# zubair-irshad/articulated-object-nerf

Measured on AMD Instinct MI355X. Metric: rays/sec (64c+128f samples), higher is better.
Workload: dtype f32; 1 GPU; sapien-single-scene vanilla NeRF full-frame render 640x480, 65 coarse + 193 fine evals/ray, 307200 rays per GPU per step, randomized=False, white_bkgd=True; rays_per_gpu=307200, evals_per_ray=258, exchange=none

## Files before the change

articulated-object-nerf_amd/_lib.py:

```python
from __future__ import annotations

import ctypes as C
import os

import torch

_PKG = os.path.dirname(os.path.abspath(__file__))
LIB_PATH = os.environ.get("AON_HIP_LIB") or os.path.join(_PKG, "libaon_hip.so")

if not os.path.exists(LIB_PATH):
    raise ImportError(
        f"{LIB_PATH} not found: the HIP kernels are the product path and there is no CPU/eager fallback. "
        "Build them with `python articulated-object-nerf_amd/build.py` (needs /opt/rocm/bin/hipcc)."
    )

lib = C.CDLL(LIB_PATH)

_p, _i, _l, _f = C.c_void_p, C.c_int, C.c_int64, C.c_float
_PATH = ([_p, _p, _p, _l]
         + [_f, _f, _i, _i]
         + [_p, _p, _l]
         + [_p] * 6
         + [_p, _l, _p])
_VANILLA, _ART, _GENERAL = [_p] * 2, [_p] * 4, [_p] * 3
# ... 18 lines not shown
    head, tail = _BWD
    vanilla = _VANILLA * 2 + head + _PER_LEVEL + tail
    art = _ART + head + _PER_LEVEL + _LATENTS + _PER_LEVEL + _LATENTS + tail
    frozen = _ART + head + _PER_LEVEL + _LATENTS + tail + _OPTS
    sigs = {"aon_render_bwd": vanilla, "aon_render_bwd_ex": vanilla + _OPTS, "aon_art_render_bwd": art, "aon_art_render_bwd_ex": art + _OPTS,
            "aon_art_render_bwd_latents": frozen, "aon_art_render_bwd_inputs": frozen + _RAY_GRADS,
            "aon_grender_bwd": _GENERAL + head + _PER_LEVEL + tail + _OPTS}
    return {name: (_i, args) for name, args in sigs.items()}


_SIGS = {
    **_path_sigs(),
    **_bwd_sigs(),
    "aon_abi_version": (_i, []),
    "aon_last_error": (C.c_char_p, []),
    "aon_raygen": (_i, [_p, _i, _i, _f, _l, _l, _p, _p, _p, _p]),
    "aon_train_loss_fwd": (_i, [_p, _p, _p, _l, _p, _p, _f, _p, _p, _p]),
    "aon_train_loss_bwd": (_i, [_p, _p, _p, _l, _p, _p, _f, _p, _p, _p, _p, _p]),
    "aon_ray_directions": (_i, [_i, _i, _f, _p, _p]),
    "aon_get_rays": (_i, [_p, _p, _l, _p, _p, _p, _p]),
    "aon_ray_radii": (_i, [_p, _p, _i, _i, _p, _p]),
    "aon_cast_rays": (_i, [_p, _p, _p, _l, _i, _p, _p]),
    "aon_sample_along_rays": (_i, [_p, _p, _l, _i, _f, _f, _p, _p, _p, _p]),
    "aon_pos_enc": (_i, [_p, _l, _i, _i, _p, _p]),
    "aon_mlp_packed_bytes": (_l, []),
    "aon_pack_vanilla_mlp": (_i, [_p, _p, _p]),
    "aon_mlp_fwd": (_i, [_p, _p, _p, _p, _p, _l, _i, _p, _p]),
    "aon_mlp_fwd_enc": (_i, [_p, _p, _p, _l, _i, _p, _p]),
    "aon_composite": (_i, [_p, _i, _p, _i, _p, _p, _l, _i, _i, _i, _p, _p, _p, _p, _p]),
    "aon_sample_pdf": (_i, [_p, _p, _l, _p, _p, _l, _l, _p, _p, _p]),
    "aon_art_packed_bytes": (_l, []),
    "aon_art_small_bytes": (_l, []),
    "aon_pack_art_mlp": (_i, [_p, _p, _p]),
    "aon_art_prepare": (_i, [_p, _p, _p, _p, _p, _p]),
    "aon_pack_art_mlp_deg": (_i, [_p, _i, _i, _i, _p, _p]),
    "aon_art_prepare_deg": (_i, [_p, _p, _p, _p, _i, _i, _i, _p, _p]),
    "aon_pack_art_mlp_bwd_deg": (_i, [_p, _i, _i, _i, _p, _p]),
    "aon_art_mlp_fwd": (_i, [_p, _p, _p, _p, _p, _p, _l, _i, _p, _p]),
    "aon_art_mlp_fwd_pos": (_i, [_p, _p, _p, _p, _l, _i, _p, _p]),
    "aon_train_plane_rows": (_l, []),
    "aon_bwd_packed_bytes": (_l, []),
    "aon_wgrad_workspace_bytes": (_l, []),
    "aon_pack_vanilla_mlp_bwd": (_i, [_p, _p, _p]),
    "aon_train_mask_bytes": (_l, [_l]),
    "aon_mlp_fwd_train": (_i, [_p, _p, _p, _p, _p, _l, _i, _p, _p, _p, _p]),
    "aon_composite_bwd": (_i, [_p, _p, _p, _p, _p, _p, _l, _i, _i, _i, _p, _p]),
    "aon_mlp_bwd_chain": (_i, [_p, _p, _p, _p, _p, _l, _p]),
    "aon_vanilla_wgrad": (_i, [_p, _p, _p, _l, _p, _p, _l, _p, _p]),
    "aon_wgrad_plan": (_i, [_i, _l, _i, _p, _i, _p]),
    "aon_wgrad_plan_segment": (_i, [_i, _l, _i, _i, _i, _p]),
    "aon_wgrad_kind_bench": (_i, [_i, _i, _p, _p, _i, _l, _p, _l, _p]),
    "aon_art_train_plane_rows": (_l, []),
    "aon_art_train_mask_bytes": (_l, [_l]),
    "aon_art_bwd_packed_bytes": (_l, []),
    "aon_pack_art_mlp_bwd": (_i, [_p, _p, _p]),
    "aon_art_mlp_fwd_train": (_i, [_p, _p, _p, _p, _p, _p, _l, _i, _p, _p, _p, _p]),
    "aon_art_bwd_chain": (_i, [_p, _p, _p, _p, _p, _p, _p, _l, _p]),
    "aon_art_wgrad": (_i, [_p, _p, _p, _p, _l, _p, _p, _p, _p, _p, _p, _p, _p, _p, _l, _p, _p]),
    "aon_art_wgrad_deg": (_i, [_p, _p, _p, _p, _l, _p, _p, _p, _p, _p, _p, _p, _p, _p, _l, _p, _i, _i, _i, _p]),
    "aon_set_bottleneck_fold": (_i, [_i]),
    "aon_get_bottleneck_fold": (_i, []),
    "aon_stream_is_folded": (_i, [_p]),
    "aon_stream_form": (_i, [_p]),
    "aon_declare_stream_form": (_i, [_p, _i]),
    "aon_adam_step": (_i, [_p, _p, _p, _p, _l, C.c_double, C.c_double, C.c_double, C.c_double, _l, _p]),
    "aon_code_library_fwd": (_i, [_p, _p, _p, _p, _p, _p]),
    "aon_code_library_bwd": (_i, [_p, _p, _p, _p, _p, _p]),
    "aon_ssim_workspace_bytes": (_l, [_i, _p, _p]),
    "aon_ssim": (_i, [_i, _p, _p, _p, _p, _p, _l, _p, _p]),
    "aon_density_grid": (_i, [_p, _p, _p, _p, _l, _l, _i, _p, _p]),
    "aon_art_density_grid": (_i, [_p, _p, _p, _p, _p, _l, _l, _i, _p, _p]),
    "aon_marching_cubes_workspace_bytes": (_l, [_p]),
    "aon_marching_cubes_count": (_i, [_p, _p, _f, _p, _l, _p, _p]),
    "aon_marching_cubes": (_i, [_p, _p, _f, _p, _p, _p, _l, _p, _l, _p, _l, _p]),
    "aon_occupancy_bytes": (_l, [_p]),
    "aon_occupancy_build": (_i, [_p, _p, _f, _i, _p, _p]),
    "aon_render_occ_workspace_bytes": (_l, [_l, _p]),
    "aon_render_stop_workspace_bytes": (_l, [_l, _p]),
    "aon_art_pack_step": (_i, [_p, _p, _p, _p, _p, _i, _i, _i, _p, _p, _p, _p, _p, _p, _p]),
    "aon_vanilla_pack_step": (_i, [_p, _p, _i, _i, _i, _p, _p, _p, _p, _p]),
    "aon_set_bwd_early_heads": (_i, [_i]),
    "aon_set_view_bias": (_i, [_i]),
    "aon_get_view_bias": (_i, []),
    "aon_view_bias": (_i, [_p, _p, _l, _p, _p]),
    "aon_set_bwd_overlap": (_i, [_i]),
    "aon_set_fwd_overlap": (_i, [_i]),
    "aon_set_fwd_merge": (_i, [_i]),
    "aon_set_bwd_merge": (_i, [_i]),
    "aon_set_wgrad_probe": (_i, [_p]),
    "aon_train_workspace_bytes": (_l, [_l, _i, _i]),
    "aon_train_scratch_bytes": (_l, [_l, _i, _i]),
    "aon_profile_begin": (_i, []),
    "aon_profile_end": (_i, [C.POINTER(C.c_double), C.POINTER(C.c_int64), C.POINTER(C.c_int64)]),
    "aon_profile_class": (_i, [_i, C.POINTER(C.c_double), C.POINTER(C.c_int64), C.POINTER(C.c_int64)]),
    "aon_composite_pdf": (_i, [_p, _p, _p, _l, _i, _i, _p, _l, _p, _p, _p, _p, _p, _p]),
    "aon_set_coarse_fusion": (_i, [_i]),
    "aon_render_workspace_bytes": (_l, [_l]),
    "aon_render_opts_init": (None, [_p]),
    "aon_pack_vanilla_mlp_deg": (_i, [_p, _i, _i, _i, _p, _p]),
    "aon_pack_vanilla_mlp_bwd_deg": (_i, [_p, _i, _i, _i, _p, _p]),
    "aon_sample_along_rays_ex": (_i, [_p, _p, _l, _i, _f, _f, _i, _f, _f, _p, _p, _p, _p]),
    "aon_composite_ex": (_i, [_p, _i, _p, _i, _p, _p, _l, _i, _i, _i, _p, _p, _p, _p, _p, _p]),
    "aon_sample_pdf_n": (_i, [_p, _p, _l, _p, _p, _l, _l, _i, _i, _i, _p, _p, _p]),
    "aon_render_workspace_bytes_ex": (_l, [_l, _p]),
    "aon_train_workspace_bytes_ex": (_l, [_l, _i, _i, _p]),
    "aon_train_scratch_bytes_ex": (_l, [_l, _i, _i, _p]),
    "aon_train_scratch_bytes_latents": (_l, [_l, _i, _p]),
    "aon_train_scratch_bytes_inputs": (_l, [_l, _i, _p]),
    "aon_mlp_geometry_init": (None, [_p]),
    "aon_gmlp_param_count": (_i, [_p]),
    "aon_gmlp_workspace_bytes": (_l, [_p, _l]),
    "aon_gmlp_fwd": (_i, [_p, _p, _p, _p, _l, _i, _p, _p, _p, _l, _p]),
    "aon_grender_workspace_bytes": (_l, [_p, _l, _p]),
    "aon_grender_train_workspace_bytes": (_l, [_p, _l, _i, _p]),
    "aon_grender_train_scratch_bytes": (_l, [_p, _l, _i, _p]),
    "aon_ray_limits_box": (_i, [_p, _p, _l, _p, _p, _p, _p, _p]),
    "aon_ray_limits_workspace_bytes": (_l, [_l]),
    "aon_ray_limits": (_i, [_p, _p, _l, _p, _p, _p, _p, _p, _p, _l, _p]),
    "aon_sample_along_rays_bounds": (_i, [_p, _p, _l, _i, _p, _p, _i, _p, _p, _p, _p]),
}


class MlpGeometryC(C.Structure):
    _fields_ = [(n, C.c_int32) for n in ("min_deg_point", "max_deg_point", "deg_view", "netdepth", "netwidth", "netdepth_condition",
                                         "netwidth_condition", "skip_layer", "input_ch", "input_ch_view", "num_rgb_channels",
                                         "num_density_channels")]


class RenderOptsC(C.Structure):
    _fields_ = [("num_coarse_samples", C.c_int32), ("num_fine_samples", C.c_int32), ("lindisp", C.c_int32),
                ("inv_near", C.c_float), ("inv_far", C.c_float), ("noise_std", C.c_float),
                ("noise_c", C.c_void_p), ("noise_f", C.c_void_p),
                ("rgb_scale", C.c_float), ("rgb_shift", C.c_float), ("sigma_bias", C.c_float),
                ("min_deg_point", C.c_int32), ("max_deg_point", C.c_int32), ("deg_view", C.c_int32)]


class OccupancyC(C.Structure):
    _fields_ = [("bits", C.c_void_p), ("cells", C.c_int64 * 3), ("lo", C.c_float * 3), ("step", C.c_float * 3)]


class RayGradsC(C.Structure):
    _fields_ = [("rays_o", C.c_void_p), ("viewdirs", C.c_void_p), ("g_rays_o", C.c_void_p), ("g_rays_d", C.c_void_p), ("g_viewdirs", C.c_void_p)]


class RayBoundsC(C.Structure):
    _fields_ = [("near_ray", C.c_void_p), ("far_ray", C.c_void_p), ("live", C.c_void_p)]


class SceneObjectC(C.Structure):
    _fields_ = [("rot", C.c_float * 9), ("centre", C.c_float * 3), ("lo", C.c_float * 3), ("hi", C.c_float * 3)]


def _ext_sigs():
    head, tail = _BWD
    return {"aon_render_bwd_inputs": (_i, _VANILLA * 2 + head + _PER_LEVEL + tail + _OPTS + _RAY_GRADS),
            "aon_train_scratch_bytes_inputs_vanilla": (_l, [_l, _i] + _OPTS)}


_EXT_SIGS = _ext_sigs()

_SCENE_SIGS = {
    "aon_scene_pairs_workspace_bytes": (_l, [_l, _i]),
    "aon_scene_pairs": (_i, [_p, _p, _p, _l] + [_p, _i] + [_p, _l] + [_p] * 8 + [_p]),
    "aon_scene_composite": (_i, [_p] * 4 + [_l, _i, _l, _i, _i, _i] + [_p] + [_p] * 5 + [_p]),
}

# ... 54 lines not shown
```

articulated-object-nerf_amd/csrc/aon_capi.hip:

```cpp
#include "aon_capi_util.h"

namespace aon {
namespace capi __attribute__((visibility("hidden"))) {

thread_local char g_err[256] = "";

int fail(int code, const char* msg) {
  std::snprintf(g_err, sizeof(g_err), "%s", msg);
  return code;
}

int check(hipError_t e, const char* where) {
  if (e == hipSuccess) return AON_OK;
  std::snprintf(g_err, sizeof(g_err), "%s: %s", where, hipGetErrorString(e));
  return AON_E_HIP_BASE - (int)e;
}

const char* const kFormsMsg = "two of the packed buffers of this call were made in different forms (aon_set_bottleneck_fold changed between the pack / prepare calls), "
                              "or one of them was never packed or declared by this process (a copy: aon_declare_stream_form)";
const char* const kNullBwdMsg = "packed_bwd is NULL (= literal planes) while the process default is the folded form: pass the transposed stream the chain ran with";

Profiler g_prof;

std::atomic<int> g_fuse_coarse{1};
std::atomic<int> g_view_bias{1};

const char* make_geo(const aon_render_opts* o, Geo& g, bool general_engine) {
  aon_render_opts d;
  aon_render_opts_init(&d);
  if (o) d = *o;
  if (d.num_coarse_samples < 2 || d.num_coarse_samples > 1023) return "num_coarse_samples must be in [2, 1023]";
  if (d.num_fine_samples < 1) return "num_fine_samples must be >= 1";
  g.Sc = d.num_coarse_samples + 1; g.nf = d.num_fine_samples; g.Sf = g.Sc + g.nf;
  g.default_sizes = g.Sc == kSc && g.Sf == kSf;
  if (!g.default_sizes && aon::sample_pdf_n_lds_bytes(g.Sc - 1, g.nf, g.Sc, nullptr) > 64 * 1024) return "num_coarse_samples / num_fine_samples too large for the per-ray LDS image";
  g.lindisp = d.lindisp != 0; g.inv_near = d.inv_near; g.inv_far = d.inv_far;
  g.noise[0] = d.noise_c; g.noise[1] = d.noise_f; g.noise_std = d.noise_std;
  g.rgb_scale = d.rgb_scale; g.rgb_shift = d.rgb_shift; g.sigma_bias = d.sigma_bias;
  g.min_deg = d.min_deg_point; g.max_deg = d.max_deg_point; g.deg_view = d.deg_view;
  if (general_engine) { g.min_deg = 0; g.max_deg = 10; g.deg_view = 4; g.other_degrees = false; return nullptr; }
  if (g.max_deg < g.min_deg || g.max_deg - g.min_deg > 10 || g.deg_view < 0 || g.deg_view > 4)
    return "the fused kernels hold up to 10 position and 4 view frequency levels (other degrees: aon_grender_*)";
  g.other_degrees = !(g.min_deg == 0 && g.max_deg == 10 && g.deg_view == 4);
  return nullptr;
}

}
}

using namespace aon::capi;

extern "C" {

int aon_abi_version(void) { return AON_ABI_VERSION; }

const char* aon_last_error(void) { return g_err; }

int aon_raygen(const float* c2w_host, int H, int W, float focal, int64_t pix_begin, int64_t pix_end, float* rays_o,
               float* viewdirs, float* rays_d, void* stream) {
  if (!c2w_host || !rays_o || !viewdirs) return fail(AON_E_INVALID, "aon_raygen: null pointer");
  if (H <= 0 || W <= 0 || !(focal > 0.f) || pix_begin < 0 || pix_end < pix_begin || pix_end > (int64_t)H * W)
    return fail(AON_E_INVALID, "aon_raygen: bad geometry");
  return check(aon::launch_raygen(c2w_host, H, W, focal, nullptr, pix_begin, pix_end, rays_o, viewdirs, rays_d,
                                  (hipStream_t)stream), "aon_raygen");
}

int aon_train_loss_fwd(const float* rgb_coarse, const float* rgb_fine, const float* target, int64_t n, const float* const* latents_host, const int* latent_len_host,
                       float reg_scale, float* stats, float* loss, void* stream) {
  if (!rgb_fine || !target || !stats || !loss) return fail(AON_E_INVALID, "aon_train_loss_fwd: null pointer");
  if (n <= 0) return fail(AON_E_INVALID, "aon_train_loss_fwd: bad size");
  for (int k = 0; k < 3 && latents_host; ++k)
    if (latents_host[k] && (!latent_len_host || latent_len_host[k] <= 0)) return fail(AON_E_INVALID, "aon_train_loss_fwd: bad latent length");
  return check(aon::launch_train_loss(false, rgb_coarse, rgb_fine, target, n, latents_host, latent_len_host, reg_scale, stats, loss, nullptr, nullptr, nullptr, nullptr,
                                      (hipStream_t)stream), "aon_train_loss_fwd");
}

int aon_train_loss_bwd(const float* rgb_coarse, const float* rgb_fine, const float* target, int64_t n, const float* const* latents_host, const int* latent_len_host,
                       float reg_scale, const float* grad_loss, float* d_rgb_coarse, float* d_rgb_fine, float* const* d_latents_host, void* stream) {
  if (!rgb_fine || !target || !grad_loss || !d_rgb_fine) return fail(AON_E_INVALID, "aon_train_loss_bwd: null pointer");
  if (n <= 0) return fail(AON_E_INVALID, "aon_train_loss_bwd: bad size");
  if ((rgb_coarse == nullptr) != (d_rgb_coarse == nullptr)) return fail(AON_E_INVALID, "aon_train_loss_bwd: coarse level input / gradient mismatch");
  for (int k = 0; k < 3 && latents_host; ++k)
    if (latents_host[k] && (!latent_len_host || latent_len_host[k] <= 0)) return fail(AON_E_INVALID, "aon_train_loss_bwd: bad latent length");
  return check(aon::launch_train_loss(true, rgb_coarse, rgb_fine, target, n, latents_host, latent_len_host, reg_scale, nullptr, nullptr, grad_loss, d_rgb_coarse, d_rgb_fine,
                                      d_latents_host, (hipStream_t)stream), "aon_train_loss_bwd");
}

int aon_view_bias(const void* packed, const float* viewdirs, int64_t n_rays, float* view_bias, void* stream) {
  if (n_rays < 0) return fail(AON_E_INVALID, "aon_view_bias: bad size");
  if (n_rays == 0) return AON_OK;
  if (!packed || !viewdirs || !view_bias) return fail(AON_E_INVALID, "aon_view_bias: null pointer");
  if (aon::stream_form(packed) != aon::kFormFolded) return fail(AON_E_INVALID, "aon_view_bias: the stream was packed in the literal form (aon_set_bottleneck_fold)");
  return check(aon::launch_view_bias(static_cast<const char*>(packed), viewdirs, n_rays, view_bias, (hipStream_t)stream), "aon_view_bias");
}

int aon_ray_directions(int H, int W, float focal, float* directions, void* stream) {
  if (H <= 0 || W <= 0 || !(focal > 0.f) || !directions) return fail(AON_E_INVALID, "aon_ray_directions: bad argument");
  return check(aon::launch_ray_directions(H, W, focal, directions, (hipStream_t)stream), "aon_ray_directions");
}

int aon_get_rays(const float* directions, const float* c2w_host, int64_t n, float* rays_o, float* viewdirs, float* rays_d,
                 void* stream) {
  if (n < 0) return fail(AON_E_INVALID, "aon_get_rays: bad size");
  if (n == 0) return AON_OK;
  if (!directions || !c2w_host || !rays_o || !viewdirs) return fail(AON_E_INVALID, "aon_get_rays: null pointer");
  return check(aon::launch_raygen(c2w_host, 1, (int)(n > INT32_MAX ? INT32_MAX : n), 1.0f, directions, 0, n, rays_o, viewdirs,
                                  rays_d, (hipStream_t)stream), "aon_get_rays");
}
// ... 489 lines not shown
int64_t aon_marching_cubes_workspace_bytes(const int64_t* dims3_host) {
  if (const char* msg = mc_dims_bad(dims3_host)) return fail(AON_E_INVALID, (std::string("aon_marching_cubes_workspace_bytes: ") + msg).c_str());
  return aon::mc_workspace_bytes(dims3_host);
}
int aon_marching_cubes_count(const float* grid, const int64_t* dims3_host, float level, void* workspace, int64_t workspace_bytes, int64_t* counts2_host,
                             void* stream) {
  if (const char* msg = mc_dims_bad(dims3_host)) return fail(AON_E_INVALID, (std::string("aon_marching_cubes_count: ") + msg).c_str());
  if (!grid || !workspace || !counts2_host) return fail(AON_E_INVALID, "aon_marching_cubes_count: null pointer");
  if (reinterpret_cast<uintptr_t>(workspace) & 15) return fail(AON_E_INVALID, "aon_marching_cubes_count: workspace is not 16-byte aligned");
  if (workspace_bytes < aon::mc_workspace_bytes(dims3_host)) return fail(AON_E_WORKSPACE, "aon_marching_cubes_count: workspace too small");
  if (int rc = check(aon::launch_mc_count(grid, dims3_host, level, workspace, (hipStream_t)stream, counts2_host), "aon_marching_cubes_count"); rc != AON_OK)
    return rc;
  if (counts2_host[0] > INT32_MAX)
    return fail(AON_E_INVALID, "aon_marching_cubes_count: more than 2^31 - 1 vertices (faces hold int32 vertex ids): use a coarser grid");
  return AON_OK;
}
int aon_marching_cubes(const float* grid, const int64_t* dims3_host, float level, const float* lo3_host, const float* step3_host, void* workspace,
                       int64_t workspace_bytes, float* verts, int64_t n_verts, int32_t* faces, int64_t n_faces, void* stream) {
  if (const char* msg = mc_dims_bad(dims3_host)) return fail(AON_E_INVALID, (std::string("aon_marching_cubes: ") + msg).c_str());
  if (!grid || !workspace || !lo3_host || !step3_host) return fail(AON_E_INVALID, "aon_marching_cubes: null pointer");
  if (n_verts < 0 || n_faces < 0 || n_verts > INT32_MAX) return fail(AON_E_INVALID, "aon_marching_cubes: bad output size");
  if ((n_verts > 0 && !verts) || (n_faces > 0 && !faces)) return fail(AON_E_INVALID, "aon_marching_cubes: null output");
  if (reinterpret_cast<uintptr_t>(workspace) & 15) return fail(AON_E_INVALID, "aon_marching_cubes: workspace is not 16-byte aligned");
  if (workspace_bytes < aon::mc_workspace_bytes(dims3_host)) return fail(AON_E_WORKSPACE, "aon_marching_cubes: workspace too small");
  return check(aon::launch_mc(grid, dims3_host, level, lo3_host, step3_host, workspace, verts, n_verts, faces, n_faces, (hipStream_t)stream),
               "aon_marching_cubes");
}

int aon_profile_begin(void) {
  std::lock_guard<std::mutex> lk(g_prof.mu);
  g_prof.on = true; g_prof.used = 0; g_prof.recs.clear();
  for (int c = 0; c < kNumClasses; ++c) g_prof.units[c] = 0;
  return AON_OK;
}

int aon_profile_end(double* mlp_ms, int64_t* mlp_launches, int64_t* mlp_samples) {
  std::lock_guard<std::mutex> lk(g_prof.mu);
  g_prof.on = false;
  for (int c = 0; c < kNumClasses; ++c) { g_prof.last_ms[c] = 0.0; g_prof.last_launches[c] = 0; g_prof.last_units[c] = g_prof.units[c]; }
  for (const auto& r : g_prof.recs) {
    hipError_t e = hipEventSynchronize(r.stop);
    if (e != hipSuccess) return check(e, "aon_profile_end");
    float ms = 0.f;
    e = hipEventElapsedTime(&ms, r.start, r.stop);
    if (e != hipSuccess) return check(e, "aon_profile_end");
    g_prof.last_ms[r.cls] += ms;
    g_prof.last_launches[r.cls] += 1;
  }
  if (mlp_ms) *mlp_ms = g_prof.last_ms[kMlpFwd];
  if (mlp_launches) *mlp_launches = g_prof.last_launches[kMlpFwd];
  if (mlp_samples) *mlp_samples = g_prof.last_units[kMlpFwd];
  g_prof.used = 0; g_prof.recs.clear();
  return AON_OK;
}

int aon_profile_class(int cls, double* ms, int64_t* launches, int64_t* units) {
  if (cls < 0 || cls >= kNumClasses) return fail(AON_E_INVALID, "aon_profile_class: unknown kernel class");
  std::lock_guard<std::mutex> lk(g_prof.mu);
  if (ms) *ms = g_prof.last_ms[cls];
  if (launches) *launches = g_prof.last_launches[cls];
  if (units) *units = g_prof.last_units[cls];
  return AON_OK;
}

int aon_set_bottleneck_fold(int on) {
  aon::set_fold_default(on);
  return AON_OK;
}
int aon_get_bottleneck_fold(void) { return aon::fold_default(); }
int aon_stream_is_folded(const void* packed) { return aon::stream_form(packed) == aon::kFormFolded ? 1 : 0; }
int aon_stream_form(const void* packed) { return aon::stream_form(packed); }
int aon_declare_stream_form(const void* packed, int form) {
  if (!packed || (form != aon::kFormLiteral && form != aon::kFormFolded)) return fail(AON_E_INVALID, "aon_declare_stream_form: null pointer or form not 0 / 1");
  aon::set_stream_form(packed, form);
  return AON_OK;
}

int aon_set_view_bias(int on) {
  g_view_bias.store(on ? 1 : 0, std::memory_order_relaxed);
  return AON_OK;
}

int aon_get_view_bias(void) { return g_view_bias.load(std::memory_order_relaxed); }

int64_t aon_art_packed_bytes(void) { return aon::art_stream_bytes(); }
int64_t aon_art_small_bytes(void) { return aon::art_small_bytes(); }

int aon_pack_art_mlp(const float* const* params_host, void* packed, void* stream) {
  return aon_pack_art_mlp_deg(params_host, 0, 10, 4, packed, stream);
}
int aon_pack_art_mlp_deg(const float* const* params_host, int min_deg_point, int max_deg_point, int deg_view, void* packed, void* stream) {
  if (const char* bad = art_degrees_ok(min_deg_point, max_deg_point, deg_view)) return fail(AON_E_INVALID, bad);
  if (!params_host || !packed) return fail(AON_E_INVALID, "aon_pack_art_mlp: null pointer");
  for (int i = 0; i < 40; ++i)
    if (!params_host[i]) return fail(AON_E_INVALID, "aon_pack_art_mlp: null parameter pointer");
  if (reinterpret_cast<uintptr_t>(packed) & 15) return fail(AON_E_INVALID, "aon_pack_art_mlp: packed must be 16-byte aligned");
  return check(aon::launch_pack_art(params_host, static_cast<float*>(packed), (hipStream_t)stream, max_deg_point - min_deg_point, deg_view),
               "aon_pack_art_mlp");
}

int aon_art_prepare(const float* const* params_host, const float* shape, const float* appearance, const float* articulation,
                    void* small, void* stream) {
  return aon_art_prepare_deg(params_host, shape, appearance, articulation, 0, 10, 4, small, stream);
}
int aon_art_prepare_deg(const float* const* params_host, const float* shape, const float* appearance, const float* articulation,
                        int min_deg_point, int max_deg_point, int deg_view, void* small, void* stream) {
  if (const char* bad = art_degrees_ok(min_deg_point, max_deg_point, deg_view)) return fail(AON_E_INVALID, bad);
  if (!params_host || !shape || !appearance || !articulation || !small) return fail(AON_E_INVALID, "aon_art_prepare: null pointer");
  for (int i = 0; i < 40; ++i)
    if (!params_host[i]) return fail(AON_E_INVALID, "aon_art_prepare: null parameter pointer");
  if (reinterpret_cast<uintptr_t>(small) & 15) return fail(AON_E_INVALID, "aon_art_prepare: small must be 16-byte aligned");
  return check(aon::launch_prepare_art(params_host, shape, appearance, articulation, static_cast<float*>(small), (hipStream_t)stream, min_deg_point,
                                       max_deg_point - min_deg_point, deg_view), "aon_art_prepare");
}

int aon_art_pack_step(const float* const* params_coarse_host, const float* const* params_fine_host, const float* shape, const float* appearance,
                      const float* articulation, int min_deg_point, int max_deg_point, int deg_view, void* packed_coarse, void* small_coarse,
                      void* packed_bwd_coarse, void* packed_fine, void* small_fine, void* packed_bwd_fine, void* stream_) {
  if (const char* bad = art_degrees_ok(min_deg_point, max_deg_point, deg_view)) return fail(AON_E_INVALID, bad);
  if (!params_coarse_host || !params_fine_host || !shape || !appearance || !articulation || !packed_coarse || !small_coarse || !packed_fine || !small_fine)
    return fail(AON_E_INVALID, "aon_art_pack_step: null pointer");
  for (int i = 0; i < 40; ++i)
    if (!params_coarse_host[i] || !params_fine_host[i]) return fail(AON_E_INVALID, "aon_art_pack_step: null parameter pointer");
  for (const void* p : {(const void*)packed_coarse, (const void*)small_coarse, (const void*)packed_fine, (const void*)small_fine, (const void*)packed_bwd_coarse, (const void*)packed_bwd_fine})
    if (reinterpret_cast<uintptr_t>(p) & 15) return fail(AON_E_INVALID, "aon_art_pack_step: buffers must be 16-byte aligned");
  hipStream_t stream = (hipStream_t)stream_;
  const int Lp = max_deg_point - min_deg_point, Lv = deg_view;
  const float* const* P[2] = {params_coarse_host, params_fine_host};
  float* fwd[2] = {static_cast<float*>(packed_coarse), static_cast<float*>(packed_fine)};
  float* sm[2] = {static_cast<float*>(small_coarse), static_cast<float*>(small_fine)};
  float* bwd[2] = {static_cast<float*>(packed_bwd_coarse), static_cast<float*>(packed_bwd_fine)};
  const int form = aon::fold_default();
  const bool folded = form == aon::kFormFolded;
  if (folded) {
    aon::FoldGemm jobs[4];
    int n = 0;
    for (int l = 0; l < 2; ++l) jobs[n++] = aon::art_fold_job_fwd(P[l], fwd[l], Lv);
    for (int l = 0; l < 2; ++l)
      if (bwd[l]) jobs[n++] = aon::art_fold_job_bwd(P[l], bwd[l], Lv);
    if (int rc = check(aon::launch_fold_gemms(jobs, n, stream), "aon_art_pack_step")) return rc;
  }
  if (int rc = check(aon::launch_pack_prepare_art2(P, shape, appearance, articulation, fwd, sm, stream, min_deg_point, Lp, Lv, form), "aon_art_pack_step")) return rc;
  if (bwd[0] && bwd[1]) return check(aon::launch_pack_art_bwd2(P, bwd, stream, Lp, Lv, form), "aon_art_pack_step");
  for (int l = 0; l < 2; ++l)
    if (bwd[l])
      if (int rc = check(aon::launch_pack_art_bwd(P[l], bwd[l], stream, Lp, Lv, folded), "aon_art_pack_step")) return rc;
  return AON_OK;
}

int aon_art_mlp_fwd(const void* packed, const void* small, const float* rays_o, const float* rays_d, const float* viewdirs,
                    const float* t_vals, int64_t n_rays, int S, float* raw, void* stream) {
  if (n_rays < 0 || S < 1) return fail(AON_E_INVALID, "aon_art_mlp_fwd: bad size");
  if (n_rays == 0) return AON_OK;
  if (!packed || !small || !rays_o || !rays_d || !viewdirs || !t_vals || !raw) return fail(AON_E_INVALID, "aon_art_mlp_fwd: null pointer");
  if (forms_differ(packed, small)) return fail(AON_E_INVALID, kFormsMsg);
  MlpTimer timer((hipStream_t)stream, n_rays * S);
  return check(aon::launch_art_mlp_fwd(static_cast<const char*>(packed), static_cast<const float*>(small), rays_o, rays_d, viewdirs,
                                       t_vals, n_rays, S, raw, (hipStream_t)stream), "aon_art_mlp_fwd");
}

int aon_art_mlp_fwd_pos(const void* packed, const void* small, const float* pos, const float* viewdirs_enc, int64_t n_rays, int S,
                        float* raw, void* stream) {
  if (n_rays < 0 || S < 1) return fail(AON_E_INVALID, "aon_art_mlp_fwd_pos: bad size");
  if (n_rays == 0) return AON_OK;
  if (!packed || !small || !pos || !viewdirs_enc || !raw) return fail(AON_E_INVALID, "aon_art_mlp_fwd_pos: null pointer");
  if (forms_differ(packed, small)) return fail(AON_E_INVALID, kFormsMsg);
// ... 6 lines not shown
```

articulated-object-nerf_amd/csrc/aon_capi_render.hip:

```cpp
#include "aon_capi_util.h"

using namespace aon::capi;

namespace {

struct Ws {
  float* t_c;
  float* w_c;
  float* t_f;
  float* raw;
  float* coords; float* enc; float* venc;
  float* vbias;
  char* occ;
  char* stop;
  int64_t bytes;
};

Ws carve(char* base, int64_t n, const Geo& g, bool occ = false, bool stop = false) {
  Ws w{};
  int64_t off = 0;
  w.t_c = reinterpret_cast<float*>(base + off); off += align_up(n * g.Sc * 4, 256);
  w.w_c = reinterpret_cast<float*>(base + off); off += align_up(n * g.Sc * 4, 256);
  w.t_f = reinterpret_cast<float*>(base + off); off += align_up(n * g.Sf * 4, 256);
  w.raw = reinterpret_cast<float*>(base + off); off += align_up(n * g.Sf * 16, 256);
  if (g.other_degrees) {
    w.coords = reinterpret_cast<float*>(base + off); off += align_up(n * g.Sf * 12, 256);
    w.enc = reinterpret_cast<float*>(base + off); off += align_up(n * g.Sf * (int64_t)aon::kPosEnc * 4, 256);
    w.venc = reinterpret_cast<float*>(base + off); off += align_up(n * (int64_t)aon::kViewEnc * 4, 256);
  } else {
    w.vbias = reinterpret_cast<float*>(base + off); off += align_up(n * (int64_t)aon::kCondWidth * 4, 256);
  }
  if (occ) { w.occ = base + off; off += aon::occ_list_bytes(n * g.Sf); }
  if (stop) { w.stop = base + off; off += aon::occ_stop_state_bytes(n); }
  w.bytes = off;
  return w;
}

}

extern "C" {

static int64_t workspace_query(int64_t n_rays, const aon_render_opts* opts, bool occ, bool stop) {
  Geo g;
  if (const char* bad = make_geo(opts, g)) return fail(AON_E_INVALID, bad);
  if (n_rays < 1) n_rays = 1;
  if (occ && n_rays > INT32_MAX / g.Sf) n_rays = INT32_MAX / g.Sf;
  return carve(nullptr, n_rays, g, occ, stop).bytes;
}
int64_t aon_render_workspace_bytes_ex(int64_t n_rays, const aon_render_opts* opts) { return workspace_query(n_rays, opts, false, false); }
int64_t aon_render_workspace_bytes(int64_t n_rays) { return aon_render_workspace_bytes_ex(n_rays, nullptr); }


struct NetRef {
  bool articulated;
  const void* packed;
  const float* small;
};
struct Nets { NetRef c, f; };
static Nets vanilla_nets(const void* packed_coarse, const void* packed_fine) {
  return {{false, packed_coarse, nullptr}, {false, packed_fine, nullptr}};
}
static Nets art_nets(const void* packed_coarse, const void* small_coarse, const void* packed_fine, const void* small_fine) {
  return {{true, packed_coarse, static_cast<const float*>(small_coarse)}, {true, packed_fine, static_cast<const float*>(small_fine)}};
}

struct OccCtx {
  aon::OccGrid grid;
  int64_t* tally;
  bool rounds;
  float tau_stop;
  int R;
  int32_t* stop_dev;
};

static hipError_t launch_net(const NetRef& net, const float* o, const float* d, const float* v, const float* t, int64_t n, int S,
                             float* raw, hipStream_t stream, const Geo* g = nullptr, const Ws* w = nullptr, const OccCtx* occ = nullptr,
                             int level = 0, const uint8_t* live = nullptr) {
  if (g && g->other_degrees) {
    if (hipError_t e = aon::launch_cast_rays(t, o, d, n, S, w->coords, stream); e != hipSuccess) return e;
    if (hipError_t e = aon::launch_pos_enc(w->coords, n * S, g->min_deg, g->max_deg, w->enc, stream, aon::kPosEnc, 10); e != hipSuccess) return e;
    if (hipError_t e = aon::launch_pos_enc(v, n, 0, g->deg_view, w->venc, stream, aon::kViewEnc, 4); e != hipSuccess) return e;
    MlpTimer timer(stream, n * S);
    return aon::launch_mlp_fwd_enc(static_cast<const char*>(net.packed), w->enc, w->venc, n, S, raw, stream);
  }
  const float* vbias = nullptr;
  if (w && w->vbias && g_view_bias.load(std::memory_order_relaxed) != 0 && aon::stream_form(net.packed) == aon::kFormFolded) {
    const hipError_t e = net.articulated ? aon::launch_art_view_bias(static_cast<const char*>(net.packed), net.small, v, n, w->vbias, stream)
                                         : aon::launch_view_bias(static_cast<const char*>(net.packed), v, n, w->vbias, stream);
    if (e != hipSuccess) return e;
    vbias = w->vbias;
  }
  const int* idx = nullptr;
  const int64_t* count = nullptr;
  auto compact = [&](int s0, int s1, const int* stop) {
    const int64_t starts[2] = {0, n};
    const aon::OccCompact c{&occ->grid, starts, 1, S, s0, s1, o, d, t, live, stop};
    return aon::launch_occ_compact(c, raw, w->occ, (n * S + 1023) / 1024, occ->tally ? occ->tally + level : nullptr, &idx, &count, stream);
  };
  if (occ && occ->rounds) {
    if (hipError_t e = aon::launch_occ_stop_init(w->stop, n, S, stream); e != hipSuccess) return e;
    const int R = occ->R < S ? occ->R : S;
    const aon::ActParams ap = g->act(net.articulated, level, 0);
    for (int s0 = 0; s0 < S; s0 += R) {
      const int s1 = s0 + R < S ? s0 + R : S;
      if (hipError_t e = compact(s0, s1, aon::occ_stop_state(w->stop, n).stop); e != hipSuccess) return e;
      {
        MlpTimer timer(stream, n * (s1 - s0));
        const hipError_t e = net.articulated ? aon::launch_art_mlp_fwd_gather(static_cast<const char*>(net.packed), net.small, o, d, v, t, n, S, raw, stream,
                                                                              vbias, idx, count, n * (s1 - s0))
                                             : aon::launch_mlp_fwd_gather(static_cast<const char*>(net.packed), o, d, v, t, n, S, raw, stream, vbias, idx,
                                                                          count, n * (s1 - s0));
        if (e != hipSuccess) return e;
      }
      if (s1 < S)
        if (hipError_t e = aon::launch_occ_depth(raw, t, d, n, S, s0, s1, ap, occ->tau_stop, w->stop, stream); e != hipSuccess) return e;
    }
    return hipSuccess;
  }
  if (occ) {
    if (hipError_t e = compact(0, S, nullptr); e != hipSuccess) return e;
    MlpTimer timer(stream, n * S);
    if (net.articulated)
      return aon::launch_art_mlp_fwd_gather(static_cast<const char*>(net.packed), net.small, o, d, v, t, n, S, raw, stream, vbias, idx, count);
    return aon::launch_mlp_fwd_gather(static_cast<const char*>(net.packed), o, d, v, t, n, S, raw, stream, vbias, idx, count);
  }
  MlpTimer timer(stream, n * S);
  if (net.articulated)
    return aon::launch_art_mlp_fwd(static_cast<const char*>(net.packed), net.small, o, d, v, t, n, S, raw, stream, vbias);
  return aon::launch_mlp_fwd(static_cast<const char*>(net.packed), o, d, v, t, n, S, raw, stream, vbias);
}

static int render_impl(const char* who, const NetRef& coarse, const NetRef& fine, const PathCall& c, const OccCtx* occ = nullptr) {
  Geo g;
  if (const char* bad = make_geo(c.opts, g)) return fail(AON_E_INVALID, bad);
  if (int rc = path_call_check(who, c, g, true)) return rc == kPathEmpty ? AON_OK : rc;
  const int64_t n_rays = c.n_rays;
  const int num_levels = c.num_levels;
  const hipStream_t stream = c.stream;
  auto bad = [&](const char* what) { return fail(AON_E_INVALID, (std::string(who) + ": " + what).c_str()); };
  if (!coarse.packed || (num_levels == 2 && !fine.packed)) return bad("null pointer");
  if (coarse.articulated && (!coarse.small || (num_levels == 2 && !fine.small))) return bad("null latent block");
  if (coarse.articulated && (forms_differ(coarse.packed, coarse.small) || (num_levels == 2 && forms_differ(fine.packed, fine.small)))) return fail(AON_E_INVALID, kFormsMsg);
  const bool art = coarse.articulated;
  if (art) g.other_degrees = false;
  const bool fuse_coarse = num_levels == 2 && g.default_sizes && g_fuse_coarse.load(std::memory_order_relaxed) != 0;
  const bool with_occ = occ != nullptr;
  const bool with_stop = with_occ && occ->rounds;

  int64_t chunk = n_rays;
  if (with_occ && chunk > INT32_MAX / g.Sf) chunk = INT32_MAX / g.Sf;
  if (carve(nullptr, chunk, g, with_occ, with_stop).bytes > c.workspace_bytes) {
    const int64_t per_ray = (int64_t)(g.Sc + g.Sc + g.Sf + 4 * g.Sf + (g.other_degrees ? (3 + aon::kPosEnc) * g.Sf + aon::kViewEnc : aon::kCondWidth) +
                                      (with_occ ? g.Sf + 2 * (g.Sf / 1024 + 1) : 0) + (with_stop ? 2 : 0)) * 4;
    const int64_t slack = (g.other_degrees ? 7 * 256 : 5 * 256) + (with_occ ? 4 * 256 : 0) + (with_stop ? 2 * 256 : 0);
    chunk = (c.workspace_bytes - slack) / per_ray;
    while (chunk > 0 && carve(nullptr, chunk, g, with_occ, with_stop).bytes > c.workspace_bytes) --chunk;
    if (chunk < 1) return fail(AON_E_WORKSPACE, with_stop ? "render: workspace smaller than aon_render_stop_workspace_bytes(1)"
                                                : with_occ ? "render: workspace smaller than aon_render_occ_workspace_bytes(1)"
                                                         : "render: workspace smaller than aon_render_workspace_bytes(1)");
  }
  const Ws w = carve(static_cast<char*>(c.workspace), chunk, g, with_occ, with_stop);
  if (with_occ && occ->tally) {
    if (int rc = check(hipMemsetAsync(occ->tally, 0, 2 * sizeof(int64_t), stream), who); rc != AON_OK) return rc;
  }

  for (int64_t r0 = 0; r0 < n_rays; r0 += chunk) {
    const int64_t n = n_rays - r0 < chunk ? n_rays - r0 : chunk;
    const float* o = c.rays_o + r0 * 3;
    const float* d = c.rays_d + r0 * 3;
    const float* v = c.viewdirs + r0 * 3;
    const float* uu = c.u_stride ? c.u + r0 * c.u_stride : c.u;
    const float* near_ray = c.bounds ? c.bounds->near_ray + r0 : nullptr;
    const float* far_ray = c.bounds ? c.bounds->far_ray + r0 : nullptr;
    const uint8_t* live = c.bounds && c.bounds->live ? c.bounds->live + r0 : nullptr;
    int rc;
    {
      KTimer timer(kSampleT, stream, n);
      rc = check(aon::launch_sample_along_rays(o, d, n, g.Sc, c.near_, c.far_, c.t_rand ? c.t_rand + r0 * g.Sc : nullptr, w.t_c, nullptr, stream,
                                               g.lindisp, g.inv_near, g.inv_far, near_ray, far_ray), who);
    }
    if (rc) return rc;
    rc = check(launch_net(coarse, o, d, v, w.t_c, n, g.Sc, w.raw, stream, &g, &w, occ, 0, live), who);
    if (rc) return rc;
    if (with_stop && occ->stop_dev) {
      rc = check(aon::launch_occ_stop_store(w.stop, 0, occ->stop_dev + r0 * 2, n, 2, stream), who);
      if (rc) return rc;
    }
    if (fuse_coarse) {
      KTimer timer(kCompositePdf, stream, n);
      rc = check(aon::launch_composite_pdf(w.raw, w.t_c, d, n, c.white_bkgd, g.act(art, 0, r0), uu, c.u_stride, c.rgb[0] + r0 * 3,
                                           c.acc[0] + r0, c.depth[0] + r0, nullptr, w.t_f, stream), who);
    } else {
      KTimer timer(kComposite, stream, n);
      rc = check(aon::launch_composite(w.raw, 4, w.raw + 3, 4, w.t_c, d, n, g.Sc, c.white_bkgd, g.act(art, 0, r0), c.rgb[0] + r0 * 3, c.acc[0] + r0,
                                       c.depth[0] + r0, num_levels == 2 ? w.w_c : nullptr, stream), who);
    }
    if (rc) return rc;
    if (num_levels == 1) continue;
    if (!fuse_coarse) {
      KTimer timer(kSamplePdf, stream, n);
      rc = check(g.default_sizes ? aon::launch_sample_pdf(nullptr, w.w_c + 1, kSc, w.t_c, uu, c.u_stride, n, nullptr, w.t_f, stream)
                                 : aon::launch_sample_pdf_n(nullptr, w.w_c + 1, g.Sc, w.t_c, uu, c.u_stride, n, g.Sc - 1, g.nf, g.Sc, nullptr,
                                                            w.t_f, stream), who);
      if (rc) return rc;
    }
    rc = check(launch_net(fine, o, d, v, w.t_f, n, g.Sf, w.raw, stream, &g, &w, occ, 1, live), who);
    if (rc) return rc;
    if (with_stop && occ->stop_dev) {
      rc = check(aon::launch_occ_stop_store(w.stop, 0, occ->stop_dev + r0 * 2 + 1, n, 2, stream), who);
      if (rc) return rc;
    }
    {
      KTimer timer(kComposite, stream, n);
      rc = check(aon::launch_composite(w.raw, 4, w.raw + 3, 4, w.t_f, d, n, g.Sf, c.white_bkgd, g.act(art, 1, r0), c.rgb[1] + r0 * 3, c.acc[1] + r0,
                                       c.depth[1] + r0, nullptr, stream), who);
    }
    if (rc) return rc;
  }
  return AON_OK;
}

int64_t aon_occupancy_bytes(const int64_t* cells3_host) {
  if (const char* msg = occ_cells_bad(cells3_host)) return fail(AON_E_INVALID, (std::string("aon_occupancy_bytes: ") + msg).c_str());
  return (cells3_host[0] * cells3_host[1] * cells3_host[2] + 31) / 32 * 4;
}
int aon_occupancy_build(const float* density, const int64_t* dims3_host, float threshold, int dilate, uint32_t* bits, void* stream) {
  if (!dims3_host) return fail(AON_E_INVALID, "aon_occupancy_build: null dims");
  const int64_t cells[3] = {dims3_host[0] - 1, dims3_host[1] - 1, dims3_host[2] - 1};
  if (const char* msg = occ_cells_bad(cells)) return fail(AON_E_INVALID, (std::string("aon_occupancy_build: every dimension must be >= 2; ") + msg).c_str());
  if (dilate < 0 || dilate > 8) return fail(AON_E_INVALID, "aon_occupancy_build: dilate must be in [0, 8]");
  if (threshold != threshold) return fail(AON_E_INVALID, "aon_occupancy_build: threshold is NaN");
  if (!density || !bits) return fail(AON_E_INVALID, "aon_occupancy_build: null pointer");
  return check(aon::launch_occ_build(density, dims3_host, threshold, dilate, bits, (hipStream_t)stream), "aon_occupancy_build");
}
static const char* occ_opts_bad(const aon_render_opts* opts, bool art, const float* t_rand) {
  Geo g;
  if (const char* bad = make_geo(opts, g)) return bad;
  if (t_rand) return "occupancy rendering is inference only: t_rand (randomized sampling) is refused";
  if (g.noise_std > 0.f && (g.noise[0] || g.noise[1])) return "occupancy rendering is inference only: density noise is refused";
  if (!art && g.other_degrees) return "occupancy rendering needs the default encoding degrees (0, 10, 4) of the vanilla network";
  return nullptr;
}
int64_t aon_render_occ_workspace_bytes(int64_t n_rays, const aon_render_opts* opts) { return workspace_query(n_rays, opts, true, false); }

// ... 140 lines not shown
```

articulated-object-nerf_amd/csrc/aon_capi_util.h:

```cpp
#pragma once
#include "../../include/aon_hip.h"
#include "aon_launch.h"

#include <atomic>
#include <cmath>
#include <cstdio>
#include <cstdlib>
#include <cstring>
#include <mutex>
#include <string>
#include <vector>

namespace aon {
namespace capi __attribute__((visibility("hidden"))) {

extern thread_local char g_err[256];

int fail(int code, const char* msg);
int check(hipError_t e, const char* where);

constexpr int kSc = 65, kSf = 193;

extern const char* const kFormsMsg;
extern const char* const kNullBwdMsg;
inline bool forms_differ(const void* a, const void* b) {
  return a && b && (aon::stream_form(a) != aon::stream_form(b) || aon::stream_form(a) == aon::kFormUnknown);
}

extern std::atomic<int> g_fuse_coarse;
extern std::atomic<int> g_view_bias;

enum KClass { kMlpFwd = AON_PROF_MLP_FWD, kBwdChain = AON_PROF_BWD_CHAIN, kWgrad = AON_PROF_WGRAD, kComposite = AON_PROF_COMPOSITE,
              kSamplePdf = AON_PROF_SAMPLE_PDF, kCompositeBwd = AON_PROF_COMPOSITE_BWD, kCompositePdf = AON_PROF_COMPOSITE_PDF, kSampleT = AON_PROF_SAMPLE_T,
              kNumClasses = AON_PROF_NUM_CLASSES };

struct Profiler {
  std::mutex mu;
  bool on = false;
  struct Rec { int cls; hipEvent_t start, stop; };
  std::vector<hipEvent_t> pool;
  size_t used = 0;
  std::vector<Rec> recs;
  int64_t units[kNumClasses] = {};
  double last_ms[kNumClasses] = {};
  int64_t last_launches[kNumClasses] = {};
  int64_t last_units[kNumClasses] = {};
};
extern Profiler g_prof;

struct KTimer {
  hipEvent_t stop = nullptr;
  hipStream_t stream;
  KTimer(int cls, hipStream_t s, int64_t units) : stream(s) {
    std::lock_guard<std::mutex> lk(g_prof.mu);
    if (!g_prof.on) return;
    while (g_prof.used + 2 > g_prof.pool.size()) {
      hipEvent_t e;
      if (hipEventCreate(&e) != hipSuccess) return;
      g_prof.pool.push_back(e);
    }
    hipEvent_t start = g_prof.pool[g_prof.used];
    stop = g_prof.pool[g_prof.used + 1];
    g_prof.used += 2;
    g_prof.recs.push_back({cls, start, stop});
    g_prof.units[cls] += units;
    (void)hipEventRecord(start, stream);
  }
  ~KTimer() { if (stop) (void)hipEventRecord(stop, stream); }
};
struct MlpTimer : KTimer {
  MlpTimer(hipStream_t s, int64_t samples) : KTimer(kMlpFwd, s, samples) {}
};

inline int64_t align_up(int64_t x, int64_t a) { return (x + a - 1) / a * a; }

struct Geo {
  int Sc, Sf, nf;
  bool default_sizes;
  int lindisp; float inv_near, inv_far;
  const float* noise[2]; float noise_std;
  float rgb_scale, rgb_shift, sigma_bias;
  int min_deg, max_deg, deg_view;
  bool other_degrees;
  int S(int l) const { return l == 0 ? Sc : Sf; }
  aon::ActParams act(bool art, int level, int64_t ray0) const {
    aon::ActParams ap{art ? AON_ACT_ARTICULATED : AON_ACT_VANILLA, rgb_scale, rgb_shift, sigma_bias, nullptr, noise_std};
    if (noise[level] && noise_std > 0.f) ap.noise = noise[level] + ray0 * S(level);
    return ap;
  }
};

const char* make_geo(const aon_render_opts* o, Geo& g, bool general_engine = false);

inline const char* occ_cells_bad(const int64_t* cells3) {
  if (!cells3) return "null cell counts";
  for (int a = 0; a < 3; ++a)
    if (cells3[a] < 1 || cells3[a] > (int64_t)1 << 24) return "every cell count must be in [1, 2^24]";
  if (cells3[0] > ((int64_t)1 << 40) / cells3[1] / cells3[2]) return "grid too large (more than 2^40 cells)";
  return nullptr;
}
inline const char* occ_grid_bad(const aon_occupancy* occ, aon::OccGrid& G) {
  if (!occ || !occ->bits) return "null occupancy grid";
  if (const char* msg = occ_cells_bad(occ->cells)) return msg;
  G.bits = occ->bits;
  for (int a = 0; a < 3; ++a) {
    if (!std::isfinite(occ->lo[a]) || !std::isfinite(occ->step[a]) || !(occ->step[a] > 0.f)) return "occupancy lo must be finite and step finite and > 0";
    G.cells[a] = occ->cells[a]; G.lo[a] = occ->lo[a]; G.step[a] = occ->step[a];
    const float span = (float)occ->cells[a] * occ->step[a];
    G.hi[a] = occ->lo[a] + span;
    if (!std::isfinite(G.hi[a])) return "occupancy box not finite";
  }
  return nullptr;
}
// ... 58 lines not shown
```

articulated-object-nerf_amd/csrc/aon_launch.h:

```cpp
#pragma once
#include "aon_common.h"
#include "aon_fold.h"

namespace aon {

int num_cus();
hipError_t launch_pack_vanilla(const float* const* params, float* packed, hipStream_t stream, int pos_levels = 10, int view_levels = 4, bool fold_done = false);
void vanilla_fold_jobs_fwd(const float* const* params, float* packed, int view_levels, FoldGemm jobs[2]);
hipError_t launch_mlp_fwd(const char* packed, const float* rays_o, const float* rays_d, const float* viewdirs,
                          const float* t_vals, int64_t n_rays, int S, float* raw, hipStream_t stream, const float* view_bias = nullptr);
hipError_t launch_view_bias(const char* packed, const float* viewdirs, int64_t n_rays, float* out, hipStream_t stream);
hipError_t launch_view_bias_raw(const float* chunk, const float* bias_vec, const float* viewdirs, int64_t n_rays, float* out, hipStream_t stream);
hipError_t launch_mlp_fwd_enc(const char* packed, const float* samples_enc, const float* viewdirs_enc, int64_t n_rays,
                              int S, float* raw, hipStream_t stream);
hipError_t launch_mlp_fwd_gather(const char* packed, const float* rays_o, const float* rays_d, const float* viewdirs, const float* t_vals,
                                 int64_t n_rays, int S, float* raw, hipStream_t stream, const float* view_bias, const int* idx, const int64_t* count,
                                 int64_t max_listed = 0);
hipError_t launch_mlp_fwd_train(const char* packed, const float* rays_o, const float* rays_d, const float* viewdirs,
                                const float* t_vals, int64_t n_rays, int S, float* raw, float* planes, void* masks,
                                hipStream_t stream, int64_t np_total = 0, const float* view_bias = nullptr);
hipError_t launch_mlp_fwd_train2(const TrainSeg* segs, int nsegs, hipStream_t stream);
hipError_t launch_mlp_fwd_train_enc(const char* packed, const float* samples_enc, const float* viewdirs_enc, int64_t n_rays, int S, float* raw,
                                    float* planes, void* masks, hipStream_t stream, int64_t np_total = 0);
hipError_t launch_density_grid(const char* packed, const int64_t* dims, const float* lo, const float* step, int64_t g_begin, int64_t g_end,
                               int act, float* out, hipStream_t stream);

int64_t art_stream_bytes();
int64_t art_small_bytes();
hipError_t launch_pack_art(const float* const* params, float* packed, hipStream_t stream, int pos_levels = 10, int view_levels = 4, bool fold_done = false);
FoldGemm art_fold_job_fwd(const float* const* params, float* packed, int view_levels);
hipError_t launch_prepare_art(const float* const* params, const float* shape, const float* app, const float* art,
                              float* small, hipStream_t stream, int min_deg = 0, int pos_levels = 10, int view_levels = 4);
hipError_t launch_pack_prepare_art2(const float* const* const params[2], const float* shape, const float* app, const float* art, float* const packed[2],
                                    float* const small[2], hipStream_t stream, int min_deg, int pos_levels, int view_levels, int form);
hipError_t launch_art_mlp_fwd(const char* packed, const float* small, const float* rays_o, const float* rays_d,
                              const float* viewdirs, const float* t_vals, int64_t n_rays, int S, float* raw,
                              hipStream_t stream, const float* view_bias = nullptr);
hipError_t launch_art_view_bias(const char* packed, const float* small, const float* viewdirs, int64_t n_rays, float* out, hipStream_t stream);
hipError_t launch_art_mlp_fwd_pos(const char* packed, const float* small, const float* pos, const float* viewdirs_enc,
                                  int64_t n_rays, int S, float* raw, hipStream_t stream);
hipError_t launch_art_mlp_fwd_gather(const char* packed, const float* small, const float* rays_o, const float* rays_d, const float* viewdirs,
                                     const float* t_vals, int64_t n_rays, int S, float* raw, hipStream_t stream, const float* view_bias,
                                     const int* idx, const int64_t* count, int64_t max_listed = 0);
hipError_t launch_art_mlp_fwd_train(const char* packed, const float* small, const float* rays_o, const float* rays_d,
                                    const float* viewdirs, const float* t_vals, int64_t n_rays, int S, float* raw, float* planes,
                                    void* masks, hipStream_t stream, int64_t np_total = 0, const float* view_bias = nullptr);
hipError_t launch_art_mlp_fwd_train2(const TrainSeg* segs, int nsegs, hipStream_t stream);
hipError_t launch_art_density_grid(const char* packed, const float* small, const int64_t* dims, const float* lo, const float* step,
                                   int64_t g_begin, int64_t g_end, int act, float* out, hipStream_t stream);

struct WgLayerDesc;
struct HeadDesc;
struct HeadOut;
struct ReduceArgs;

struct WgAux {
  hipStream_t stream;
  hipEvent_t fork, join;
};

enum : int { kWgAll = 0, kWgEarly = 1, kWgRest = 2 };

struct VanillaWgDeferred;
struct ArtWgDeferred;
constexpr int kVanillaWgDeferredBytes = 4096;
constexpr int kArtWgDeferredBytes = 4096;

hipError_t launch_composite_bwd(const float* raw, const float* t_vals, const float* dirs, const float* g_rgb, const float* g_acc,
                                const float* g_depth, int64_t n_rays, int S, int white_bkgd, const ActParams& ap, float* d_raw,
                                hipStream_t stream);
void vanilla_fold_jobs_bwd(const float* const* params, float* packed, int view_size, FoldGemm jobs[2]);
hipError_t launch_pack_vanilla_bwd(const float* const* params, float* packed, hipStream_t stream, int pos_size = 63, int view_size = 27, bool fold_done = false);
int64_t bwd_stream_bytes();
hipError_t launch_mlp_bwd_chain(const char* packed_bwd, const char* packed_fwd, const float* d_raw, const void* masks,
                                float* dplanes, int64_t Np, hipStream_t stream);
hipError_t launch_mlp_bwd_chain2(const ChainSeg* segs, int nsegs, hipStream_t stream);
int64_t wgrad_workspace_bytes();
float* wgrad_fold_tmp(float* ws);
void set_wgrad_probe(long long* buf);
hipError_t run_wgrad_plan(const WgLayerDesc* layers, int nlayers, const HeadDesc* heads, int nheads, const HeadOut* outs, const int* out_head, int nouts,
                          const float* planes, const float* dplanes, int rows_total, int64_t Np, float* ws, hipStream_t stream, const WgAux* aux,
                          int phase, int n_early, hipEvent_t wait_first, ReduceArgs* defer_reduce, int* defer_blocks);
hipError_t launch_wgrad_reduce2(const ReduceArgs& a0, int n0, const ReduceArgs& a1, int n1, hipStream_t stream);
hipError_t launch_wgrad_kind_bench(int kind, int nlayers, const float* planes, const float* dplanes, int rows_total, int64_t Np, float* ws,
                                   float* out_scratch, hipStream_t stream);
hipError_t launch_vanilla_wgrad(const float* planes, const float* dplanes, const float* d_raw, int64_t Np, float* const* grads,
                                float* ws, hipStream_t stream, const WgAux* aux, const void* packed_bwd, int phase = kWgAll, hipEvent_t wait_first = nullptr,
                                VanillaWgDeferred* defer = nullptr);
hipError_t launch_vanilla_wgrad_post2(const VanillaWgDeferred* d0, const VanillaWgDeferred* d1, hipStream_t stream);
int vanilla_wgrad_deferred_bytes();
int wgrad_plan_describe(bool art, int64_t Np, int cus, int32_t* out6, int max_jobs, int64_t* ws_bytes);
int wgrad_plan_segment(bool art, int64_t Np, int cus, int j, int wg, int32_t* begin_end);

// ... 115 lines not shown
```

articulated-object-nerf_amd/csrc/aon_mlp.hip:

```cpp
#include "aon_pass.h"

namespace aon {

struct VanillaNet {
  static constexpr int kSlotBytes = kPairSlotBytes;
  static constexpr bool kPair = true;
  static constexpr int kNumChunks = aon::kNumChunks;
  static constexpr int chunk_bytes(int c) { return aon::chunk_bytes(c); }
};
struct VanillaFoldNet {
  static constexpr int kSlotBytes = kPairSlotBytes;
  static constexpr bool kPair = true;
  static constexpr int kNumChunks = aon::kNumChunksF;
  static constexpr int chunk_bytes(int c) { return aon::chunk_bytes_f(c); }
};
struct VanillaFoldVbNet {
  static constexpr int kSlotBytes = kPairSlotBytes;
  static constexpr bool kPair = true;
  static constexpr int kNumChunks = aon::kNumChunksF - 1;
  static constexpr int chunk_bytes(int c) { return aon::chunk_bytes_f(c < kChFView ? c : c + 1); }
  static constexpr int skip_before(int c) { return c == kChFView ? kSmallChunkBytes : 0; }
};

struct PackArgs {
  const float* p[kNumVanillaParams];
};

template <bool FOLD>
__global__ void pack_vanilla_kernel(PackArgs a, float* __restrict__ packed, int L, int Lv) {
  const int P = 3 + 6 * L, V = 3 + 6 * Lv;
  const int64_t idx = (int64_t)blockIdx.x * blockDim.x + threadIdx.x;
  constexpr int64_t stream_floats = kStreamBytes / 4;
  constexpr int64_t used_floats = FOLD ? kStreamBytesF / 4 : stream_floats;
  const float* Wf = packed + kFoldTmpOff / 4;
  if (idx >= stream_floats + kSmallFloats) return;
  if (idx >= used_floats && idx < stream_floats) {
    if (idx >= used_floats + 128 * 256 + 128) packed[idx] = 0.f;
    return;
  }
  if (idx >= stream_floats) {
    const int s = (int)(idx - stream_floats);
    float v = 0.f;
    if (s < kSmBiasBott) v = a.p[2 * (s >> 8) + 1][s & 255];
    else if (s < kSmBiasView) v = a.p[19][s - kSmBiasBott];
    else if (s < kSmWSigma) v = FOLD ? Wf[128 * 256 + s - kSmBiasView] : a.p[17][s - kSmBiasView];
    else if (s < kSmWRgb) v = a.p[20][s - kSmWSigma];
    else if (s < kSmBSigma) v = a.p[22][s - kSmWRgb];
    else if (s < kSmBRgb) v = a.p[21][0];
    else if (s < kSmBRgb + 3) v = a.p[23][s - kSmBRgb];
    packed[idx] = v;
    return;
  }
  int c, r, nt;
  constexpr int nbig = FOLD ? kChFView : kNumBigChunks;
  if (idx < (int64_t)nbig * (kBigChunkBytes / 4)) {
    c = (int)(idx / (kBigChunkBytes / 4)); r = (int)(idx % (kBigChunkBytes / 4)); nt = 8;
  } else {
    const int64_t i2 = idx - (int64_t)nbig * (kBigChunkBytes / 4);
    c = nbig + (int)(i2 / (kSmallChunkBytes / 4)); r = (int)(i2 % (kSmallChunkBytes / 4)); nt = 4;
    if constexpr (FOLD) c = c == kChFView ? kChView + 8 : c - 1 + (kChView - kChFView);
  }
  const int cc = r & 3, lane = (r >> 2) & 63, rest = r >> 8;
  const int tp = rest % nt, q = rest / nt;
  const int h = lane >> 5, row = 32 * tp + (lane & 31);
  const float* W; int ld, n_out = 256, col;
  const int hid_col = 8 * q + 4 * h + cc;
  auto pcol = [&](int c63) { return c63 < 0 ? -1 : pos_col_in(c63, L); };
  auto vcol = [&](int c27) { return c27 < 0 ? -1 : view_col_in(c27, Lv); };
  if (c < kChL1) { W = a.p[0]; ld = P; col = pcol(posenc_col(c, q, cc, h)); }
  else if (c < kChL5) { const int l = 1 + (c - kChL1) / 8; W = a.p[2 * l]; ld = 256; col = 32 * ((c - kChL1) % 8) + hid_col; }
  else if (c < kChL5 + 8) { W = a.p[10]; ld = 256 + P; col = 32 * (c - kChL5) + hid_col; }
  else if (c < kChL6) { W = a.p[10]; ld = 256 + P; col = pcol(posenc_col(c - kChL5 - 8, q, cc, h)); if (col >= 0) col += 256; }
  else if (c < kChL7) { W = a.p[12]; ld = 256; col = 32 * (c - kChL6) + hid_col; }
  else if (c < kChBott) { W = a.p[14]; ld = 256; col = 32 * (c - kChL7) + hid_col; }
  else if (c < kChView) { W = a.p[18]; ld = 256; col = 32 * (c - kChBott) + hid_col; }
  else if (c < kChView + 8) {
    W = a.p[16]; ld = 256 + V; n_out = kCondWidth; col = 32 * (c - kChView) + hid_col;
    if constexpr (FOLD) { W = Wf; ld = 256; }
  }
  else { W = a.p[16]; ld = 256 + V; n_out = kCondWidth; col = vcol(viewenc_col(q, cc, h)); if (col >= 0) col += 256; }
  packed[idx] = (col >= 0 && row < n_out) ? W[(int64_t)row * ld + col] : 0.f;
}

struct MlpSeg {
  const char* packed;
  const float* rays_o;
  const float* rays_d;
  const float* viewdirs;
  const float* t_vals;
  const float* samples_enc;
  const float* viewdirs_enc;
  float* raw;
  int64_t total;
  int S;
  int npass;
  union {
    float* planes;
    const int* gather_idx;
  };
  union {
    u32x4* masks;
    const int64_t* gather_count;
  };
  int64_t Np;
  const float* view_bias;
  static constexpr bool kPerCallBlock = false;
};
struct MlpArgs {
  MlpSeg seg[2];
  int npass_total;
};
__host__ __device__ __forceinline__ const char* seg_stream(const MlpSeg& s) { return s.packed; }
__device__ __forceinline__ const float* seg_small(const MlpSeg& s) { return reinterpret_cast<const float*>(s.packed + kStreamBytes); }

constexpr int kLdsBytes = kRingBytes + (int)kSmallBytes;

struct VanillaTrunk {
  static constexpr int kL0 = kChL0, kL1 = kChL1, kL5 = kChL5, kL6 = kChL6, kL7 = kChL7;
  static constexpr int kBias = kSmBias, kWSigma = kSmWSigma, kBSigma = kSmBSigma, kMask0 = 0;
  static constexpr int plane(int l) { return plane_h(l); }
};

template <bool ENC_IN_KERNEL, bool TRAIN, bool FOLD, bool VB = false, bool GATHER = false>
__global__ void __launch_bounds__(256) mlp_fwd_kernel(MlpArgs args) {
  static_assert(FOLD || !VB, "the per-ray view bias belongs to the folded form");
  static_assert(!GATHER || (ENC_IN_KERNEL && !TRAIN), "the occupancy list serves the inference kernel on in-kernel encodings");
  using Net = std::conditional_t<VB, VanillaFoldVbNet, std::conditional_t<FOLD, VanillaFoldNet, VanillaNet>>;
  const int tid = threadIdx.x;
  const int lane = tid & 63, wave = tid >> 6;
  const int m = lane & 31, h = lane >> 5;
  const int wave_s = __builtin_amdgcn_readfirstlane(wave);

  run_passes<Net, kSmallFloats, GATHER>(args, [&](const MlpSeg& sg, int pass, Pipe& p, const float* sm, int64_t listed = 0) __attribute__((always_inline)) {
    int64_t g = (int64_t)pass * 128 + wave * 32 + m;
    bool valid;
    int64_t gc;
    if constexpr (GATHER) {
      valid = g < listed;
      g = gc = sg.gather_idx[valid ? g : listed - 1];
    } else {
      valid = g < sg.total;
      gc = valid ? g : sg.total - 1;
    }
    const int64_t ray = gc / sg.S;

    f32x16 E[2], V;
    float x[3] = {0.f, 0.f, 0.f}, vd[3] = {0.f, 0.f, 0.f};
    if constexpr (ENC_IN_KERNEL) {
      const float t = sg.t_vals[gc];
#pragma unroll
      for (int a = 0; a < 3; ++a) {
        x[a] = __fadd_rn(sg.rays_o[ray * 3 + a], __fmul_rn(t, sg.rays_d[ray * 3 + a]));
        vd[a] = sg.viewdirs[ray * 3 + a];
      }
      encode_pos(x, h, E);
      if constexpr (!VB || TRAIN) encode_view(vd, h, V);
    } else {
      load_pos_enc(sg.samples_enc + gc * kPosEnc, h, E);
      if constexpr (!VB || TRAIN) load_view_enc(sg.viewdirs_enc + ray * kViewEnc, h, V);
    }
    int ray32 = (int)ray;
    (void)ray32;

    PlaneIO io{};
    unsigned moff = 0;
    if constexpr (TRAIN) { io = make_plane_io(sg.planes, kPlRows, (int64_t)pass * 4 + wave_s, m, h); moff = mask_lane_off(pass, tid); }
    if constexpr (TRAIN) {
      store_pos_enc_plane(E, io, kPlE, h);
      store_view_enc_plane(V, io, kPlVE, h);
    }
    FwdTaps<TRAIN, MlpSeg> taps{sg, io, moff};
    f32x16 X[8], Y[8], Z[4];
    auto reread_enc = [&]() {
      if constexpr (TRAIN && !ENC_IN_KERNEL) {
        int64_t gq = gc;
        asm volatile("" : "+v"(gq));
        load_pos_enc(sg.samples_enc + gq * kPosEnc, h, E);
      }
    };
    auto l7_side = [&](auto plain) {
      if constexpr (VB) {
        asm volatile("" : "+v"(ray32));
        return view_bias_side(plain, sg.view_bias + (int64_t)ray32 * kCondWidth + 4 * h, Z);
      } else {
        return plain;
      }
    };
    const float sigma = trunk_fwd<Net, VanillaTrunk>(p, E, X, Y, sm, h, taps, reread_enc, l7_side);
    constexpr int kChV = FOLD ? kChFView : kChView;
    auto reencode_view = [&]() {
      if constexpr (TRAIN && ENC_IN_KERNEL) {
        asm volatile("" : "+v"(vd[0]), "+v"(vd[1]), "+v"(vd[2]));
        encode_view(vd, h, V);
      }
      if constexpr (TRAIN && !ENC_IN_KERNEL) {
        int64_t rq = ray;
        asm volatile("" : "+v"(rq));
        load_view_enc(sg.viewdirs_enc + rq * kViewEnc, h, V);
      }
    };
    if constexpr (FOLD) {
      if constexpr (!VB) {
        init_bias(Z, sm + kSmBiasView, h);
        reencode_view();
        chunk_mma<Net, kChV, 4, 14>(p, V, Z);
      }
      dense_layer<Net, kChV + (VB ? 0 : 1), 8, 4>(p, Y, Z, taps.consume(Y, plane_h(7), true)); taps.put_mask(7);
    } else {
      init_bias(X, sm + kSmBiasBott, h); dense_layer<Net, kChBott, 8, 8>(p, Y, X, taps.consume(Y, plane_h(7), true)); taps.put_mask(7);
      init_bias(Z, sm + kSmBiasView, h);
      dense_layer<Net, kChV, 8, 4>(p, X, Z, taps.consume(X, kPlBot, false));
      reencode_view();
      chunk_mma<Net, kChV + 8, 4, 14>(p, V, Z);
    }
    relu_tiles(Z);
    taps.burst(Z, kPlHV, 8);
    float rgb[3];
#pragma unroll
    for (int ch = 0; ch < 3; ++ch) {
      float v = head_partial<4>(Z, sm + kSmWRgb + ch * kCondWidth, h);
      rgb[ch] = v + __shfl_xor(v, 32) + sm[kSmBRgb + ch];
    }
    if (valid && h == 0) {
      f32x4 o; o[0] = rgb[0]; o[1] = rgb[1]; o[2] = rgb[2]; o[3] = sigma;
      reinterpret_cast<f32x4*>(sg.raw)[g] = o;
    }
  });
}

void vanilla_fold_jobs_fwd(const float* const* params, float* packed, int view_levels, FoldGemm jobs[2]) {
  float* Wf = packed + kFoldTmpOff / 4;
  fold_view_jobs(params[16], 256 + 3 + 6 * view_levels, params[17], params[18], params[19], Wf, Wf + 128 * 256, jobs);
}

hipError_t launch_pack_vanilla(const float* const* params, float* packed, hipStream_t stream, int pos_levels, int view_levels, bool fold_done) {
  PackArgs a;
  for (int i = 0; i < kNumVanillaParams; ++i) a.p[i] = params[i];
  const int64_t n = kStreamBytes / 4 + kSmallFloats;
  const int form = fold_default();
  set_stream_form(packed, form);
  if (form == kFormFolded) {
    if (!fold_done) {
      FoldGemm jobs[2];
      vanilla_fold_jobs_fwd(params, packed, view_levels, jobs);
      if (hipError_t e = launch_fold_gemms(jobs, 2, stream); e != hipSuccess) return e;
    }
    pack_vanilla_kernel<true><<<dim3((unsigned)((n + 255) / 256)), dim3(256), 0, stream>>>(a, packed, pos_levels, view_levels);
  } else {
    pack_vanilla_kernel<false><<<dim3((unsigned)((n + 255) / 256)), dim3(256), 0, stream>>>(a, packed, pos_levels, view_levels);
  }
  return hipGetLastError();
}

int num_cus() {
  static std::atomic<int> cache[kMaxDevices];
  int dev = 0;
  if (hipGetDevice(&dev) != hipSuccess) return -1;
  if (dev < 0 || dev >= kMaxDevices) return -1;
  int cus = cache[dev].load(std::memory_order_relaxed);
  if (cus == 0) {
    hipDeviceProp_t prop;
    if (hipGetDeviceProperties(&prop, dev) != hipSuccess) return -1;
    cus = prop.multiProcessorCount;
    cache[dev].store(cus, std::memory_order_relaxed);
  }
  return cus;
}

template <bool ENC, bool TRAIN, bool FOLD, bool VB = false, bool GATHER = false>
static hipError_t launch_mlp_tf(const MlpArgs& args, hipStream_t stream) {
  static DeviceOnce lds_once;
  return launch_persistent(&mlp_fwd_kernel<ENC, TRAIN, FOLD, VB, GATHER>, kLdsBytes, args.npass_total, lds_once, stream, args);
}

template <bool ENC, bool TRAIN, bool GATHER = false>
static hipError_t launch_mlp_t(const MlpArgs& args, hipStream_t stream) {
  const int form = agreed_form(args);
  if (form == kFormUnknown) return hipErrorInvalidValue;
  if (args.seg[0].view_bias != nullptr) {
    if constexpr (ENC) return launch_mlp_tf<ENC, TRAIN, true, true, GATHER>(args, stream);
    else return hipErrorInvalidValue;
  }
  return form == kFormFolded ? launch_mlp_tf<ENC, TRAIN, true, false, GATHER>(args, stream)
                             : launch_mlp_tf<ENC, TRAIN, false, false, GATHER>(args, stream);
}

__global__ __launch_bounds__(256) void view_bias_kernel(const float* chunk, const float* bias_vec, const float* viewdirs, int64_t n_rays, float* out) {
  __shared__ float enc[8][2][16];
  const int tid = threadIdx.x;
  const int64_t ray0 = (int64_t)blockIdx.x * 8;
  if (tid < 16) {
    const int64_t ray = ray0 + (tid >> 1);
    if (ray < n_rays) {
      float vd[3] = {viewdirs[ray * 3], viewdirs[ray * 3 + 1], viewdirs[ray * 3 + 2]};
      f32x16 V;
      encode_view(vd, tid & 1, V);
#pragma unroll
      for (int r = 0; r < 16; ++r) enc[tid >> 1][tid & 1][r] = V[r];
    }
  }
  const int row = tid & 127, tp = row >> 5;
  const float bias = bias_vec[row];
  float w[14][2];
#pragma unroll
  for (int r = 0; r < 14; ++r)
#pragma unroll
    for (int hh = 0; hh < 2; ++hh) w[r][hh] = chunk[((((r >> 2) * 4 + tp) * 64 + hh * 32 + (row & 31)) << 2) + (r & 3)];
  __syncthreads();
  for (int k = tid >> 7; k < 8; k += 2) {
    const int64_t ray = ray0 + k;
    if (ray >= n_rays) break;
    float acc = bias;
#pragma unroll
    for (int r = 0; r < 14; ++r) {
      acc = __builtin_fmaf(w[r][0], enc[k][0][r], acc);
      acc = __builtin_fmaf(w[r][1], enc[k][1][r], acc);
    }
    out[ray * kCondWidth + row] = acc;
  }
}

hipError_t launch_view_bias_raw(const float* chunk, const float* bias_vec, const float* viewdirs, int64_t n_rays, float* out, hipStream_t stream) {
  if (n_rays <= 0) return hipSuccess;
  view_bias_kernel<<<dim3((unsigned)((n_rays + 7) / 8)), dim3(256), 0, stream>>>(chunk, bias_vec, viewdirs, n_rays, out);
  return hipGetLastError();
}

hipError_t launch_view_bias(const char* packed, const float* viewdirs, int64_t n_rays, float* out, hipStream_t stream) {
  if (stream_form(packed) != kFormFolded) return hipErrorInvalidValue;
  return launch_view_bias_raw(reinterpret_cast<const float*>(packed + chunk_offset_f(kChFView)), reinterpret_cast<const float*>(packed + kStreamBytes) + kSmBiasView,
                              viewdirs, n_rays, out, stream);
}

hipError_t launch_mlp_fwd(const char* packed, const float* rays_o, const float* rays_d, const float* viewdirs,
                          const float* t_vals, int64_t n_rays, int S, float* raw, hipStream_t stream, const float* view_bias) {
  MlpArgs args{};
  fill_seg(args.seg[0], TrainSeg{packed, nullptr, rays_o, rays_d, viewdirs, t_vals, n_rays, S, raw, nullptr, nullptr, 0, view_bias});
  finish_segs(args, 1);
  return launch_mlp_t<true, false>(args, stream);
}

hipError_t launch_mlp_fwd_gather(const char* packed, const float* rays_o, const float* rays_d, const float* viewdirs, const float* t_vals,
                                 int64_t n_rays, int S, float* raw, hipStream_t stream, const float* view_bias, const int* idx, const int64_t* count,
                                 int64_t max_listed) {
  MlpArgs args{};
  MlpSeg& a = args.seg[0];
  fill_seg(a, TrainSeg{packed, nullptr, rays_o, rays_d, viewdirs, t_vals, n_rays, S, raw, nullptr, nullptr, 0, view_bias});
  if (max_listed > 0) a.npass = (int)((max_listed + 127) / 128);
  a.gather_idx = idx; a.gather_count = count;
  finish_segs(args, 1);
  return launch_mlp_t<true, false, true>(args, stream);
}

hipError_t launch_mlp_fwd_train(const char* packed, const float* rays_o, const float* rays_d, const float* viewdirs,
                                const float* t_vals, int64_t n_rays, int S, float* raw, float* planes, void* masks,
                                hipStream_t stream, int64_t np_total, const float* view_bias) {
  const TrainSeg one{packed, nullptr, rays_o, rays_d, viewdirs, t_vals, n_rays, S, raw, planes, masks, np_total, view_bias};
  return launch_mlp_fwd_train2(&one, 1, stream);
}

hipError_t launch_mlp_fwd_train2(const TrainSeg* segs, int nsegs, hipStream_t stream) {
  if (nsegs < 1 || nsegs > 2) return hipErrorInvalidValue;
  MlpArgs args{};
  for (int i = 0; i < nsegs; ++i) fill_seg(args.seg[i], segs[i]);
  finish_segs(args, nsegs);
  return launch_mlp_t<true, true>(args, stream);
}

hipError_t launch_mlp_fwd_train_enc(const char* packed, const float* samples_enc, const float* viewdirs_enc, int64_t n_rays, int S, float* raw,
                                    float* planes, void* masks, hipStream_t stream, int64_t np_total) {
  MlpArgs args{};
  fill_seg(args.seg[0], TrainSeg{packed, nullptr, nullptr, nullptr, nullptr, nullptr, n_rays, S, raw, planes, masks, np_total});
  args.seg[0].samples_enc = samples_enc; args.seg[0].viewdirs_enc = viewdirs_enc;
  finish_segs(args, 1);
  return launch_mlp_t<false, true>(args, stream);
}

hipError_t launch_mlp_fwd_enc(const char* packed, const float* samples_enc, const float* viewdirs_enc,
                              int64_t n_rays, int S, float* raw, hipStream_t stream) {
  MlpArgs args{};
  fill_seg(args.seg[0], TrainSeg{packed, nullptr, nullptr, nullptr, nullptr, nullptr, n_rays, S, raw, nullptr, nullptr, 0});
  args.seg[0].samples_enc = samples_enc; args.seg[0].viewdirs_enc = viewdirs_enc;
  finish_segs(args, 1);
  return launch_mlp_t<false, false>(args, stream);
}

struct VanillaTrunkNet {
  static constexpr int kSlotBytes = kPairSlotBytes;
  static constexpr bool kPair = true;
  static constexpr int kNumChunks = kChBott;
  static constexpr int chunk_bytes(int) { return kBigChunkBytes; }
};


__global__ void __launch_bounds__(256) density_grid_kernel(GridArgs args) {
  const int lane = threadIdx.x & 63, wave = threadIdx.x >> 6;
  const int m = lane & 31, h = lane >> 5;
  run_passes_one<VanillaTrunkNet, kSmallFloats>(args.packed, reinterpret_cast<const float*>(args.packed + kStreamBytes), args.npass,
                                                [&](int pass, Pipe& p, const float* sm) __attribute__((always_inline)) {
    const int64_t l0 = (int64_t)pass * 128 + wave * 32;
    const int64_t l = l0 + m;
    float x[3];
    grid_point(args, l < args.total ? l : args.total - 1, x);
    f32x16 E[2], X[8], Y[8];
    encode_pos(x, h, E);
    NoTaps taps;
    const float sigma = trunk_fwd<VanillaTrunkNet, VanillaTrunk>(p, E, X, Y, sm, h, taps);
    grid_store(args.out, l0, args.total, lane, grid_activation(sigma, args.act));
  });
}

hipError_t launch_density_grid(const char* packed, const int64_t* dims, const float* lo, const float* step, int64_t g_begin, int64_t g_end,
                               int act, float* out, hipStream_t stream) {
  if (stream_form(packed) == kFormUnknown) return hipErrorInvalidValue;
  static DeviceOnce lds_once;
  const GridArgs a = make_grid_args(packed, nullptr, dims, lo, step, g_begin, g_end, act, out);
  return launch_persistent(&density_grid_kernel, kLdsBytes, a.npass, lds_once, stream, a);
}

}
```

articulated-object-nerf_amd/csrc/aon_occ.hip:

```cpp
#include "aon_launch.h"
#include "../../include/aon_hip_scene.h"
#include "aon_occ_lookup.h"
#include "aon_ray_core.h"

namespace aon {

constexpr int kOccTile = 1024;
constexpr int kOccThreads = 256;
constexpr int kOccPer = kOccTile / kOccThreads;
constexpr int kOccWaves = kOccThreads / 64;

__global__ __launch_bounds__(kOccThreads) void occ_build_kernel(const float* __restrict__ dens, int64_t nx, int64_t ny, int64_t nz, float thr, int r,
                                                                uint32_t* __restrict__ bits, int64_t ncells, int64_t nwords) {
  const int64_t cx = nx - 1, cy = ny - 1, cz = nz - 1;
  const int64_t c = (int64_t)blockIdx.x * kOccThreads + threadIdx.x;
  bool occ = false;
  if (c < ncells) {
    const int64_t i = c / (cy * cz), rem = c - i * (cy * cz), j = rem / cz, k = rem - j * cz;
    const int64_t i0 = i - r > 0 ? i - r : 0, i1 = (i + r < cx - 1 ? i + r : cx - 1) + 1;
    const int64_t j0 = j - r > 0 ? j - r : 0, j1 = (j + r < cy - 1 ? j + r : cy - 1) + 1;
    const int64_t k0 = k - r > 0 ? k - r : 0, k1 = (k + r < cz - 1 ? k + r : cz - 1) + 1;
    for (int64_t pi = i0; pi <= i1 && !occ; ++pi)
      for (int64_t pj = j0; pj <= j1 && !occ; ++pj) {
        const float* row = dens + (pi * ny + pj) * nz;
// ... 1 lines not shown
          if (!(row[pk] <= thr)) { occ = true; break; }
      }
  }
  const uint64_t b = __ballot(occ);
  const int lane = threadIdx.x & 63;
  const int64_t word = (c - lane) / 32 + (lane >> 5);
  if ((lane & 31) == 0 && word < nwords) bits[word] = (uint32_t)(lane ? b >> 32 : b);
}

hipError_t launch_occ_build(const float* dens, const int64_t* dims, float thr, int dilate, uint32_t* bits, hipStream_t stream) {
  const int64_t ncells = (dims[0] - 1) * (dims[1] - 1) * (dims[2] - 1);
  const int64_t nwords = (ncells + 31) / 32;
  const int64_t blocks = (ncells + kOccThreads - 1) / kOccThreads;
  occ_build_kernel<<<dim3((unsigned)blocks), dim3(kOccThreads), 0, stream>>>(dens, dims[0], dims[1], dims[2], thr, dilate, bits, ncells, nwords);
  return hipGetLastError();
}

template <int KMAX>
struct OccArgs {
  OccGrid g[KMAX];
  int64_t row0[KMAX + 1];
  int tile0[KMAX + 1];
  int K, S, s0, s1;
  const float* o; const float* d; const float* t_vals;
  const uint8_t* ray_live;
  const int* stop;
};

template <int KMAX>
__host__ __device__ __forceinline__ bool occ_dense(const OccArgs<KMAX>& a, int k) { return !a.g[k].bits && !a.ray_live && !a.stop; }

template <int KMAX>
__device__ __forceinline__ bool occ_flag(const OccArgs<KMAX>& a, int k, uint32_t q, int64_t& rec, int& local) {
  const uint32_t w = a.s1 - a.s0;
  rec = -1;
  if (q >= (uint32_t)(a.row0[k + 1] - a.row0[k]) * w) return false;
  const uint32_t row_local = q / w;
  const int i = a.s0 + (int)(q - row_local * w);
  const int64_t row = a.row0[k] + row_local;
  local = (int)row_local * a.S + i;
  rec = a.row0[k] * a.S + local;
  if (a.stop && a.stop[row] <= i) return false;
  if (a.ray_live && !a.ray_live[row]) return false;
  if (!a.g[k].bits) return true;
  const float t = a.t_vals[rec];
  float x[3];
#pragma unroll
  for (int c = 0; c < 3; ++c) x[c] = __fadd_rn(a.o[row * 3 + c], __fmul_rn(t, a.d[row * 3 + c]));
  return occ_lookup(a.g[k], x);
}

struct OccTile {
  int k;
  int64_t rec[kOccPer];
  int local[kOccPer];
  uint64_t bal[kOccPer];
  bool occ[kOccPer];
};

template <int KMAX>
__device__ __forceinline__ void occ_tile_flags(const OccArgs<KMAX>& a, OccTile& s, int (&cnt)[kOccPer][kOccWaves]) {
  s.k = 0;
  for (int j = 1; j < a.K; ++j)
    if ((int)blockIdx.x >= a.tile0[j]) s.k = j;
  const uint32_t q0 = (uint32_t)((int)blockIdx.x - a.tile0[s.k]) * kOccTile + threadIdx.x;
#pragma unroll
  for (int r = 0; r < kOccPer; ++r) {
    s.occ[r] = occ_flag(a, s.k, q0 + r * kOccThreads, s.rec[r], s.local[r]);
    s.bal[r] = __builtin_amdgcn_ballot_w64(s.occ[r]);
    if ((threadIdx.x & 63) == 0) cnt[r][threadIdx.x >> 6] = __builtin_popcountll(s.bal[r]);
  }
  __syncthreads();
}

template <int KMAX>
__global__ __launch_bounds__(kOccThreads) void occ_mark_kernel(OccArgs<KMAX> a, f32x4* __restrict__ raw, int* __restrict__ tile_counts) {
  __shared__ int cnt[kOccPer][kOccWaves];
  OccTile s;
  occ_tile_flags(a, s, cnt);
  f32x4 sentinel;
  sentinel[0] = 0.f; sentinel[1] = 0.f; sentinel[2] = 0.f; sentinel[3] = -__builtin_huge_valf();
#pragma unroll
  for (int r = 0; r < kOccPer; ++r)
    if (s.rec[r] >= 0 && !s.occ[r]) raw[s.rec[r]] = sentinel;
  if (threadIdx.x == 0) {
    int tot = 0;
#pragma unroll
    for (int r = 0; r < kOccPer; ++r)
#pragma unroll
      for (int w = 0; w < kOccWaves; ++w) tot += cnt[r][w];
    tile_counts[blockIdx.x] = tot;
  }
}

template <int KMAX>
__global__ __launch_bounds__(kOccThreads) void occ_scan_kernel(OccArgs<KMAX> a, const int* __restrict__ tile_counts, int* __restrict__ offs,
                                                               int64_t* __restrict__ counts, int64_t* __restrict__ tally) {
  __shared__ int64_t red[kOccWaves];
  for (int k = 0; k < a.K; ++k) {
    const int64_t total = (occ_dense(a, k) ? (a.row0[k + 1] - a.row0[k]) * (a.s1 - a.s0) : 0) +
                          block_scan_counts(tile_counts + a.tile0[k], a.tile0[k + 1] - a.tile0[k], offs + a.tile0[k], red);
    if (threadIdx.x == 0) {
      counts[k] = total;
      if (tally) tally[k] += total;
    }
  }
}

template <int KMAX>
__global__ __launch_bounds__(kOccThreads) void occ_emit_kernel(OccArgs<KMAX> a, const int* __restrict__ offs, int* __restrict__ idx) {
  __shared__ int cnt[kOccPer][kOccWaves];
  OccTile s;
  occ_tile_flags(a, s, cnt);
  const int lane = threadIdx.x & 63, wave = threadIdx.x >> 6;
  const uint64_t below = lane == 0 ? 0ull : (~0ull >> (64 - lane));
  int* list = idx + a.row0[s.k] * a.S;
  int run = offs[blockIdx.x];
#pragma unroll
  for (int r = 0; r < kOccPer; ++r) {
    int before = run;
#pragma unroll
    for (int w = 0; w < kOccWaves; ++w) {
      if (w < wave) before += cnt[r][w];
      run += cnt[r][w];
    }
    if (s.occ[r]) list[before + __builtin_popcountll(s.bal[r] & below)] = s.local[r];
  }
}

struct OccLists {
  int* idx; int* tile_counts; int* offs; int64_t* counts;
  int64_t bytes;
};
static OccLists occ_carve(char* ws, int64_t total, int64_t tile_cap, int K) {
  auto up = [](int64_t b) { return (b + 255) / 256 * 256; };
  const int64_t o1 = up(total * 4), o2 = o1 + up(tile_cap * 4), o3 = o2 + up(tile_cap * 4);
  return {reinterpret_cast<int*>(ws), reinterpret_cast<int*>(ws + o1), reinterpret_cast<int*>(ws + o2), reinterpret_cast<int64_t*>(ws + o3),
          o3 + up((int64_t)K * 8)};
}
static int64_t occ_tiles(int64_t samples) { return (samples + kOccTile - 1) / kOccTile; }
int64_t occ_list_bytes(int64_t total) { return occ_carve(nullptr, total, occ_tiles(total), 1).bytes; }
int64_t scene_occ_tile_cap(int64_t pairs, int K, int S) { return pairs * S / kOccTile + K; }
int64_t scene_occ_list_bytes(int64_t pairs, int K, int S) {
  return occ_carve(nullptr, (pairs > 0 ? pairs : 1) * S, scene_occ_tile_cap(pairs, K, S), K).bytes;
}

template <int KMAX>
static hipError_t occ_compact(const OccCompact& c, float* raw, const OccLists& L, int64_t* tally, hipStream_t stream) {
  OccArgs<KMAX> a{};
  a.K = c.K; a.S = c.S; a.s0 = c.s0; a.s1 = c.s1;
  a.o = c.rays_o; a.d = c.rays_d; a.t_vals = c.t_vals; a.ray_live = c.ray_live; a.stop = c.stop;
  for (int k = 0; k < c.K; ++k) a.g[k] = c.grids[k];
  int64_t tiles = 0;
  for (int k = 0; k <= c.K; ++k) {
    a.row0[k] = c.starts[k];
    a.tile0[k] = (int)tiles;
    if (k < c.K && !occ_dense(a, k)) tiles += occ_tiles((c.starts[k + 1] - c.starts[k]) * (c.s1 - c.s0));
  }
  const dim3 grid((unsigned)tiles), block(kOccThreads);
  if (tiles > 0) {
    occ_mark_kernel<KMAX><<<grid, block, 0, stream>>>(a, reinterpret_cast<f32x4*>(raw), L.tile_counts);
    if (hipError_t e = hipGetLastError(); e != hipSuccess) return e;
  }
  if (tiles > 0 || tally) {
    occ_scan_kernel<KMAX><<<dim3(1), block, 0, stream>>>(a, L.tile_counts, L.offs, L.counts, tally);
    if (hipError_t e = hipGetLastError(); e != hipSuccess) return e;
  }
// ... 90 lines not shown
```

articulated-object-nerf_amd/ops.py:

```python
from __future__ import annotations

import collections as _collections
import ctypes as C

import torch

from . import _lib
from ._lib import check, lib

ACT_NONE, ACT_VANILLA, ACT_ARTICULATED = 0, 1, 2


def _stream() -> C.c_void_p:
    return C.c_void_p(torch.cuda.current_stream().cuda_stream)


STREAM_CACHE_ENTRIES = 8
_STREAM_CACHES: list = []


class StreamCache:

    def __init__(self, max_entries: int = STREAM_CACHE_ENTRIES, register: bool = True):
        self.max_entries = int(max_entries)
# ... 426 lines not shown
    return uu, nf


def sorted_piecewise_constant_pdf(bins, weights, u=None, num_samples: int = 128):
    b, w = _f32(bins, "bins"), _f32(weights, "weights")
    n, nb = b.shape
    if tuple(w.shape) != (n, nb - 1) or nb < 2:
        raise ValueError(f"weights must be ({n},{nb - 1}) for bins ({n},{nb})")
    uu, us = _u_args(u, n, b.device, num_samples)
    samples = torch.empty((n, num_samples), dtype=torch.float32, device=b.device)
    with torch.cuda.device(b.device):
        if (nb, num_samples) == (64, 128):
            check(lib.aon_sample_pdf(_ptr(b), _ptr(w), 63, None, _ptr(uu), us, n, _ptr(samples), None, _stream()), "aon_sample_pdf")
        else:
            check(lib.aon_sample_pdf_n(_ptr(b), _ptr(w), nb - 1, None, _ptr(uu), us, n, nb, num_samples, 0, _ptr(samples), None, _stream()),
                  "aon_sample_pdf_n")
    return samples


def sample_pdf_t_n(t_coarse, coarse_weights, num_samples: int, u=None, bins=None, force_generic=False):
    t, w = _f32(t_coarse, "t_coarse"), _f32(coarse_weights, "weights")
    n, nt = t.shape
    b = None if bins is None else _f32(bins, "bins")
    nb = nt - 1 if b is None else b.shape[1]
    if tuple(w.shape) == (n, nb + 1):
        w_ptr, w_stride = C.c_void_p(w.data_ptr() + 4), nb + 1
    elif tuple(w.shape) == (n, nb - 1):
        w_ptr, w_stride = _ptr(w), nb - 1
    else:
        raise ValueError(f"weights must be ({n},{nb + 1}) or ({n},{nb - 1})")
    uu, us = _u_args(u, n, t.device, num_samples)
    t_fine = torch.empty((n, nt + num_samples), dtype=torch.float32, device=t.device)
    with torch.cuda.device(t.device):
        check(lib.aon_sample_pdf_n(_ptr(b), w_ptr, w_stride, _ptr(t), _ptr(uu), us, n, nb, num_samples, nt, None, _ptr(t_fine), _stream()),
              "aon_sample_pdf_n")
    return t_fine


def sample_pdf_t(t_coarse, coarse_weights, u=None, bins=None):
    t = _f32(t_coarse, "t_coarse")
    w = _f32(coarse_weights, "weights")
    n = t.shape[0]
    if tuple(t.shape) != (n, 65):
        raise ValueError("t_coarse must be (n,65)")
    if tuple(w.shape) == (n, 65):
        w_ptr, w_stride = C.c_void_p(w.data_ptr() + 4), 65
    elif tuple(w.shape) == (n, 63):
        w_ptr, w_stride = _ptr(w), 63
    else:
        raise ValueError("weights must be (n,65) or (n,63)")
    b = None if bins is None else _f32(bins, "bins")
    uu, us = _u_args(u, n, t.device)
    t_fine = torch.empty((n, 193), dtype=torch.float32, device=t.device)
    with torch.cuda.device(t.device):
        check(lib.aon_sample_pdf(_ptr(b), w_ptr, w_stride, _ptr(t), _ptr(uu), us, n, None, _ptr(t_fine), _stream()), "aon_sample_pdf")
    return t_fine


def composite_pdf(raw, t_coarse, dirs, white_bkgd, act=ACT_VANILLA, u=None, want_weights=False):
    r, t, d = _f32(raw, "raw"), _f32(t_coarse, "t_coarse"), _f32(dirs, "dirs")
    n, dev = t.shape[0], t.device
    if tuple(t.shape) != (n, 65) or r.numel() != n * 65 * 4:
        raise ValueError("composite_pdf: t_coarse must be (n,65) and raw (n,65,4)")
    uu, us = _u_args(u, n, dev)
    comp = torch.empty((n, 3), dtype=torch.float32, device=dev)
    acc = torch.empty((n,), dtype=torch.float32, device=dev)
    depth = torch.empty((n,), dtype=torch.float32, device=dev)
    weights = torch.empty((n, 65), dtype=torch.float32, device=dev) if want_weights else None
    t_fine = torch.empty((n, 193), dtype=torch.float32, device=dev)
    with torch.cuda.device(dev):
        check(lib.aon_composite_pdf(_ptr(r), _ptr(t), _ptr(d), n, int(bool(white_bkgd)), act, _ptr(uu), us, _ptr(comp), _ptr(acc),
                                    _ptr(depth), _ptr(weights), _ptr(t_fine), _stream()), "aon_composite_pdf")
    return comp, acc, weights, depth, t_fine


def set_coarse_fusion(on: bool) -> None:
    check(lib.aon_set_coarse_fusion(int(bool(on))), "aon_set_coarse_fusion")


_WS_CACHE = StreamCache()
MAX_CHUNK_RAYS = 327680


def _workspace(device, n_rays: int, st=None) -> torch.Tensor:
    chunk = MAX_CHUNK_RAYS
    if st is not None and (st.min_deg_point, st.max_deg_point, st.deg_view) != (0, 10, 4):
        chunk = 65536
    need = int(lib.aon_render_workspace_bytes_ex(min(n_rays, chunk), None if st is None else C.byref(st)))
    if need < 0:
        check(need, "aon_render_workspace_bytes_ex")
    return _scratch(_WS_CACHE, device, need)


def _check_noise(noise, n, op, num_levels):
    if noise is None:
        return None
    out = []
    for lvl in range(num_levels):
        t = noise[lvl] if lvl < len(noise) else None
        if t is not None and t.numel() != n * op.S(lvl):
            raise ValueError(f"noise[{lvl}] must hold ({n},{op.S(lvl)}) values, got {tuple(t.shape)}")
        out.append(t)
    return out


def _level_outs(n, dev, num_levels):
    outs = [(torch.empty((n, 3), dtype=torch.float32, device=dev), torch.empty((n,), dtype=torch.float32, device=dev),
             torch.empty((n,), dtype=torch.float32, device=dev)) for _ in range(num_levels)]
    return outs, (outs[1] if num_levels == 2 else (None, None, None))


class _PathCall:

    def __init__(self, rays_o, rays_d, viewdirs, near, far, white_bkgd, num_levels, t_rand, u, opts, noise, per_ray=False, ray_live=None):
        o, d, v = _f32(rays_o, "rays_o"), _f32(rays_d, "rays_d"), _f32(viewdirs, "viewdirs")
        self.n, self.dev = n, dev = o.shape[0], o.device
        self.op = op = _opts(opts)
        near, far, self.bounds, bkeep = _ray_bounds(near, far, n, dev, ray_live) if per_ray else (float(near), float(far), None, ())
        tr = None if t_rand is None else _f32(t_rand, "t_rand")
        if tr is not None and tuple(tr.shape) != (n, op.Sc):
            raise ValueError(f"t_rand must be ({n},{op.Sc})")
        self.uu, us = _u_args(u, n, dev, op.num_fine_samples) if num_levels == 2 else (None, 0)
        self.outs, fine = _level_outs(n, dev, num_levels)
        self.st, self.noise_keep = op.c_struct(near, far, _check_noise(noise, n, op, num_levels))
        self._keep = (o, d, v, tr, bkeep)
        self._head = (_ptr(o), _ptr(d), _ptr(v), n, float(near), float(far), int(bool(white_bkgd)), num_levels, _ptr(tr), _ptr(self.uu), us,
                      *(_ptr(x) for x in self.outs[0]), *(_ptr(x) for x in fine))

    def args(self, ws):
        return (*self._head, _ptr(ws), ws.numel(), _stream(), C.byref(self.st))


def _render_call(name, packs, rays_o, rays_d, viewdirs, near, far, white_bkgd, num_levels, t_rand, u, opts, noise, ray_live, workspace_bytes):
    if isinstance(near, torch.Tensor) or isinstance(far, torch.Tensor) or ray_live is not None:
        return _stop_call(name + "_stop", packs, rays_o, rays_d, viewdirs, near, far, white_bkgd, None, 0.0, None, num_levels, u, opts, workspace_bytes,
                          t_rand=t_rand, noise=noise, ray_live=ray_live, want_stats=False)[0]
    pc = _PathCall(rays_o, rays_d, viewdirs, near, far, white_bkgd, num_levels, t_rand, u, opts, noise)
    ws = _workspace(pc.dev, pc.n, pc.st)
    with torch.cuda.device(pc.dev):
        check(getattr(lib, name + "_ex")(*packs, *pc.args(ws)), name)
    return pc.outs


def render_fwd(packed_coarse, packed_fine, rays_o, rays_d, viewdirs, near, far, white_bkgd, num_levels=2, t_rand=None, u=None,
               opts=None, noise=None, ray_live=None, workspace_bytes=None):
    return _render_call("aon_render_fwd", (_pk(packed_coarse), _pk(packed_fine)), rays_o, rays_d, viewdirs, near, far, white_bkgd, num_levels, t_rand, u,
                        opts, noise, ray_live, workspace_bytes)


ART_PARAM_ORDER = (
    [f"deformations_linear.{i}.{k}" for i in range(4) for k in ("weight", "bias")]
    + [f"deformation_layer.{k}" for k in ("weight", "bias")]
    + [f"pts_linears.{i}.{k}" for i in range(8) for k in ("weight", "bias")]
    + [f"views_linear.{i}.{k}" for i in range(4) for k in ("weight", "bias")]
    + [f"{m}.{k}" for m in ("bottleneck_layer", "density_layer", "rgb_layer") for k in ("weight", "bias")]
)
ART_PARAM_SHAPES = {
    "deformations_linear.0.weight": (128, 163), "deformation_layer.weight": (3, 128), "deformation_layer.bias": (3,),
    "pts_linears.0.weight": (256, 191), "pts_linears.5.weight": (256, 447), "views_linear.0.weight": (128, 411),
    "bottleneck_layer.weight": (256, 256), "bottleneck_layer.bias": (256,), "density_layer.weight": (1, 256),
    "density_layer.bias": (1,), "rgb_layer.weight": (3, 128), "rgb_layer.bias": (3,),
}
for _i in (1, 2, 3):
    ART_PARAM_SHAPES[f"deformations_linear.{_i}.weight"] = (128, 128)
    ART_PARAM_SHAPES[f"views_linear.{_i}.weight"] = (128, 128)
for _i in range(4):
    ART_PARAM_SHAPES[f"deformations_linear.{_i}.bias"] = (128,)
    ART_PARAM_SHAPES[f"views_linear.{_i}.bias"] = (128,)
for _i in (1, 2, 3, 4, 6, 7):
    ART_PARAM_SHAPES[f"pts_linears.{_i}.weight"] = (256, 256)
for _i in range(8):
    ART_PARAM_SHAPES[f"pts_linears.{_i}.bias"] = (256,)


def art_param_shapes(degrees=(0, 10, 4)) -> dict:
    lo, hi, dv = (int(x) for x in degrees)
    if not (0 <= hi - lo <= 10 and 0 <= dv <= 4 and -32 <= lo and hi <= 32):
        raise NotImplementedError(f"articulated NeRFMLP with degrees {tuple(degrees)}: the kernels hold up to 10 position and 4 view frequency levels")
    P, V = 3 + 6 * (hi - lo), 3 + 6 * dv
    shapes = dict(ART_PARAM_SHAPES)
    shapes["pts_linears.0.weight"] = (256, P + 128)
    shapes["pts_linears.5.weight"] = (256, 256 + P + 128)
    shapes["views_linear.0.weight"] = (128, 256 + V + 128)
    return shapes


def _art_param_array(params: dict, degrees=(0, 10, 4)):
    tensors = []
    shapes = ART_PARAM_SHAPES if tuple(degrees) == (0, 10, 4) else art_param_shapes(degrees)
    for name in ART_PARAM_ORDER:
        t = _f32(params[name].detach(), name)
        if tuple(t.shape) != shapes[name]:
            raise ValueError(f"{name}: shape {tuple(t.shape)} != {shapes[name]} (the articulated NeRFMLP has HIP kernels for the "
                             f"reference's default widths at degrees {tuple(degrees)})")
        tensors.append(t)
    return tensors, (C.c_void_p * len(tensors))(*[t.data_ptr() for t in tensors])


def pack_art_mlp(params: dict, out: torch.Tensor | None = None, degrees=(0, 10, 4)) -> torch.Tensor:
    tensors, arr = _art_param_array(params, degrees)
    dev = tensors[0].device
    if out is None:
        out = torch.empty(int(lib.aon_art_packed_bytes()), dtype=torch.uint8, device=dev)
    with torch.cuda.device(dev):
        check(lib.aon_pack_art_mlp_deg(arr, int(degrees[0]), int(degrees[1]), int(degrees[2]), _ptr(out), _stream()), "aon_pack_art_mlp_deg")
    return _tag(out)


def _latent(latents: dict, key: str, width: int) -> torch.Tensor:
    t = _f32(latents[key].detach(), f"latents[{key!r}]").reshape(-1)
    if t.numel() != width:
        raise ValueError(f"latents[{key!r}] must hold {width} values (one instance per call, like the reference's "
                         f"'n1 c -> (n1 n2) c' broadcast), got {tuple(latents[key].shape)}")
    return t


def art_prepare(params: dict, latents: dict, out: torch.Tensor | None = None, degrees=(0, 10, 4)) -> torch.Tensor:
    tensors, arr = _art_param_array(params, degrees)
    dev = tensors[0].device
    shape, app, art = _latent(latents, "density", 128), _latent(latents, "color", 128), _latent(latents, "articulation", 32)
    if out is None:
# ... 179 lines not shown


def pack_art_mlp_bwd(params: dict, out: torch.Tensor | None = None, degrees=(0, 10, 4)) -> torch.Tensor:
    tensors, arr = _art_param_array(params, degrees)
    dev = tensors[0].device
    if out is None:
        out = torch.empty(int(lib.aon_art_bwd_packed_bytes()), dtype=torch.uint8, device=dev)
    with torch.cuda.device(dev):
        check(lib.aon_pack_art_mlp_bwd_deg(arr, int(degrees[0]), int(degrees[1]), int(degrees[2]), _ptr(out), _stream()), "aon_pack_art_mlp_bwd_deg")
    return _tag(out)


def art_mlp_fwd_train(packed, small, rays_o, rays_d, viewdirs, t_vals, out=None):
    o, d, v, t = _f32(rays_o, "rays_o"), _f32(rays_d, "rays_d"), _f32(viewdirs, "viewdirs"), _f32(t_vals, "t_vals")
    n, S = t.shape
    Np = padded_samples(n * S)
    if out is None:
        raw = torch.empty((n, S, 4), dtype=torch.float32, device=t.device)
    else:
        raw = out
        if not (isinstance(raw, torch.Tensor) and raw.dtype == torch.float32 and tuple(raw.shape) == (n, S, 4) and raw.device == t.device
                and raw.is_contiguous()):
            raise ValueError(f"art_mlp_fwd_train: out must be a contiguous float32 ({n}, {S}, 4) tensor on {t.device}")
    planes = _new_planes(int(lib.aon_art_train_plane_rows()), Np, t.device)
    masks = torch.empty(int(lib.aon_art_train_mask_bytes(Np)), dtype=torch.uint8, device=t.device)
    with torch.cuda.device(t.device):
        check(lib.aon_art_mlp_fwd_train(_pk(packed), _pk(small), _ptr(o), _ptr(d), _ptr(v), _ptr(t), n, S, _ptr(raw), _ptr(planes), _ptr(masks), _stream()),
              "aon_art_mlp_fwd_train")
    return raw, planes, masks


def art_bwd_chain(packed_bwd, small, d_raw, masks, planes):
    dplanes = torch.empty(planes.shape, dtype=torch.float32, device=planes.device)
    Np = plane_samples(planes)
    dxp = torch.empty((Np, 4), dtype=torch.float32, device=planes.device)
    with torch.cuda.device(planes.device):
        check(lib.aon_art_bwd_chain(_pk(packed_bwd), _pk(small), _ptr(d_raw), _ptr(masks), _ptr(planes), _ptr(dplanes), _ptr(dxp), Np, _stream()),
              "aon_art_bwd_chain")
    return dplanes, dxp


def art_wgrad(planes, dplanes, d_raw, dxp, params: dict, latents: dict, degrees=(0, 10, 4), *, packed_bwd):
    if packed_bwd is None:
        raise ValueError("art_wgrad: pass packed_bwd= the transposed stream (pack_art_mlp_bwd) the backward chain of these planes ran with")
    dev = planes.device
    ws = _scratch(_WG_WS, dev, int(lib.aon_wgrad_workspace_bytes()))
    tensors, parr = _art_param_array(params, degrees)
    shape, app, art = _latent(latents, "density", 128), _latent(latents, "color", 128), _latent(latents, "articulation", 32)
    shapes = art_param_shapes(degrees)
    grads = {name: torch.empty(shapes[name], dtype=torch.float32, device=dev) for name in ART_PARAM_ORDER}
    garr = (C.c_void_p * len(ART_PARAM_ORDER))(*[grads[n].data_ptr() for n in ART_PARAM_ORDER])
    g_lat = {"density": torch.empty(128, device=dev), "color": torch.empty(128, device=dev), "articulation": torch.empty(32, device=dev)}
    with torch.cuda.device(dev):
        check(lib.aon_art_wgrad_deg(_ptr(planes), _ptr(dplanes), _ptr(d_raw), _ptr(dxp), plane_samples(planes), parr, _ptr(shape), _ptr(app),
                                    _ptr(art), garr, _ptr(g_lat["density"]), _ptr(g_lat["color"]), _ptr(g_lat["articulation"]), _ptr(ws),
                                    ws.numel(), _stream(), int(degrees[0]), int(degrees[1]), int(degrees[2]), _pk(packed_bwd)), "aon_art_wgrad_deg")
    return grads, g_lat


def set_bottleneck_fold(on: bool) -> None:
    check(lib.aon_set_bottleneck_fold(int(bool(on))), "aon_set_bottleneck_fold")


def bottleneck_fold() -> bool:
    return bool(lib.aon_get_bottleneck_fold())


def set_bwd_overlap(on: bool) -> None:
    check(lib.aon_set_bwd_overlap(2 if on == 2 else int(bool(on))), "aon_set_bwd_overlap")


def _sized(nbytes: int, what: str, device) -> torch.Tensor:
    if nbytes < 0:
        check(nbytes, what)
    return torch.empty(nbytes, dtype=torch.uint8, device=device)


def set_fwd_overlap(on: bool) -> None:
    check(lib.aon_set_fwd_overlap(int(bool(on))), "aon_set_fwd_overlap")


def set_view_bias(on: bool) -> None:
    check(lib.aon_set_view_bias(int(bool(on))), "aon_set_view_bias")


def view_bias_enabled() -> bool:
    return bool(lib.aon_get_view_bias()) and bottleneck_fold()


def view_bias(packed: torch.Tensor, viewdirs: torch.Tensor) -> torch.Tensor:
    v = _f32(viewdirs, "viewdirs")
    n = v.numel() // 3
    out = torch.empty((n, 128), dtype=torch.float32, device=v.device)
    with torch.cuda.device(v.device):
        check(lib.aon_view_bias(_pk(packed), _ptr(v), n, _ptr(out), _stream()), "aon_view_bias")
    return out


def set_bwd_early_heads(on: bool) -> None:
    check(lib.aon_set_bwd_early_heads(int(bool(on))), "aon_set_bwd_early_heads")


def set_bwd_merge(on: bool) -> None:
    check(lib.aon_set_bwd_merge(int(bool(on))), "aon_set_bwd_merge")


def set_fwd_merge(on: bool) -> None:
    check(lib.aon_set_fwd_merge(2 if on == 2 else int(bool(on))), "aon_set_fwd_merge")


_TRAIN_POOL: "_collections.OrderedDict" = _collections.OrderedDict()
_TRAIN_POOL_KEEP = 2
_TRAIN_POOL_SIZES = 6


def _pool_take(nbytes: int, what: str, device) -> torch.Tensor:
    if nbytes < 0:
        check(nbytes, what)
    dev = torch.device(device)
    if dev.type == "cuda":
        stream = torch.cuda.current_stream(dev).cuda_stream
        key = (dev.index if dev.index is not None else torch.cuda.current_device(), nbytes)
        free = _TRAIN_POOL.get(key)
        if free:
            _TRAIN_POOL.move_to_end(key)
            for i, (t, s) in enumerate(free):
                if s == stream:
                    del free[i]
                    return t
    return torch.empty(nbytes, dtype=torch.uint8, device=device)


def pool_give(t) -> None:
    if t is None or not isinstance(t, torch.Tensor) or not t.is_cuda or t.dtype != torch.uint8 or t.dim() != 1:
        return
    key = (t.device.index, t.numel())
    free = _TRAIN_POOL.setdefault(key, [])
    _TRAIN_POOL.move_to_end(key)
    if len(free) < _TRAIN_POOL_KEEP:
        free.append((t, torch.cuda.current_stream(t.device).cuda_stream))
    while len(_TRAIN_POOL) > _TRAIN_POOL_SIZES:
        _TRAIN_POOL.popitem(last=False)


def train_workspace(device, n_rays: int, articulated: bool, num_levels: int = 2, st=None) -> torch.Tensor:
    return _pool_take(int(lib.aon_train_workspace_bytes_ex(n_rays, int(articulated), num_levels, None if st is None else C.byref(st))),
                      "aon_train_workspace_bytes_ex", device)


def _train_scratch(query: str, device, *query_args, st=None) -> torch.Tensor:
    return _pool_take(int(getattr(lib, query)(*query_args, None if st is None else C.byref(st))), query, device)


def train_scratch(device, n_rays: int, articulated: bool, num_levels: int = 2, st=None) -> torch.Tensor:
    return _train_scratch("aon_train_scratch_bytes_ex", device, n_rays, int(articulated), num_levels, st=st)


def render_fwd_train(packed_c, packed_f, rays_o, rays_d, viewdirs, near, far, white_bkgd, num_levels, t_rand, u, small_c=None, small_f=None,
                     opts=None, noise=None):
    art = small_c is not None
    pc = _PathCall(rays_o, rays_d, viewdirs, near, far, white_bkgd, num_levels, t_rand, u, opts, noise, per_ray=True)
    ws = train_workspace(pc.dev, pc.n, art, num_levels, pc.st)
    packs = (_pk(packed_c), _pk(small_c), _pk(packed_f), _pk(small_f)) if art else (_pk(packed_c), _pk(packed_f))
    stem = "aon_art_render_fwd_train" if art else "aon_render_fwd_train"
    name, extra = (stem + "_ex", ()) if pc.bounds is None else (stem + "_bounds", (C.byref(pc.bounds),))
    with torch.cuda.device(pc.dev):
# ... 534 lines not shown
def occupancy_grid(density, lo, hi, threshold: float = 0.01, dilate: int = 1) -> OccupancyGrid:
    d = _f32(density, "density")
    if d.dim() != 3:
        raise ValueError(f"occupancy_grid: expected an (nx, ny, nz) density grid, got shape {tuple(d.shape)}")
    dims = list(d.shape)
    if min(dims) < 2:
        raise ValueError(f"occupancy_grid: every dimension must be >= 2 (cells = points - 1), got {dims}")
    threshold, dilate = float(threshold), int(dilate)
    if threshold != threshold or not 0 <= dilate <= 8:
        raise ValueError("occupancy_grid: threshold must not be NaN and dilate must be in [0, 8]")
    lo32, step = grid_step(dims, lo, hi)
    if not bool((step > 0).all()):
        raise ValueError(f"occupancy_grid: need lo < hi on every axis, got lo={lo}, hi={hi}")
    cells = [n - 1 for n in dims]
    nbytes = int(lib.aon_occupancy_bytes((C.c_int64 * 3)(*cells)))
    if nbytes < 0:
        check(nbytes, "aon_occupancy_bytes")
    bits = torch.empty(nbytes // 4, dtype=torch.int32, device=d.device)
    with torch.cuda.device(d.device):
        check(lib.aon_occupancy_build(_ptr(d), (C.c_int64 * 3)(*dims), C.c_float(threshold), dilate, _ptr(bits), _stream()), "aon_occupancy_build")
    return OccupancyGrid(bits, cells, lo32, step, threshold, dilate)


_OCC_WS_CACHE = StreamCache()


def _occ_workspace(device, n_rays: int, st, workspace_bytes, query="aon_render_occ_workspace_bytes"):
    if workspace_bytes is not None:
        return torch.empty(int(workspace_bytes), dtype=torch.uint8, device=device)
    need = int(getattr(lib, query)(min(n_rays, MAX_CHUNK_RAYS), C.byref(st)))
    if need < 0:
        check(need, query)
    return _scratch(_OCC_WS_CACHE, device, need)


def render_fwd_occ(packed_coarse, packed_fine, rays_o, rays_d, viewdirs, near, far, white_bkgd, grid: OccupancyGrid, num_levels=2, u=None,
                   opts=None, workspace_bytes=None, ray_live=None):
    return _stop_call("aon_render_fwd_occ", (_pk(packed_coarse), _pk(packed_fine)), rays_o, rays_d, viewdirs, near, far, white_bkgd, grid, 0.0, None,
                      num_levels, u, opts, workspace_bytes, ray_live=ray_live)


def art_render_fwd_occ(packed_c, small_c, packed_f, small_f, rays_o, rays_d, viewdirs, near, far, white_bkgd, grid: OccupancyGrid, num_levels=2,
                       u=None, opts=None, workspace_bytes=None, ray_live=None):
    return _stop_call("aon_art_render_fwd_occ", (_pk(packed_c), _pk(small_c), _pk(packed_f), _pk(small_f)), rays_o, rays_d, viewdirs, near, far,
                      white_bkgd, grid, 0.0, None, num_levels, u, opts, workspace_bytes, ray_live=ray_live)


DEFAULT_ROUND_SAMPLES = 48


def _stop_call(name, packs, rays_o, rays_d, viewdirs, near, far, white_bkgd, grid, eps, round_samples, num_levels, u, opts, workspace_bytes,
               t_rand=None, noise=None, ray_live=None, want_stats=True):
    occ_form = name.endswith("_occ")
    if not isinstance(grid, OccupancyGrid) and (occ_form or grid is not None):
        raise TypeError(f"{name}: grid must be an ops.OccupancyGrid (ops.occupancy_grid){'' if occ_form else ' or None'}, got {type(grid)}")
    if num_levels not in (1, 2):
        raise ValueError(f"{name}: num_levels must be 1 or 2")
    eps = float(eps)
    if not 0.0 <= eps < 1.0:
        raise ValueError(f"{name}: eps must be in [0, 1), got {eps}")
    R = DEFAULT_ROUND_SAMPLES if round_samples is None else int(round_samples)
    if R < 1:
        raise ValueError(f"{name}: round_samples must be >= 1, got {R}")
    per_ray = isinstance(near, torch.Tensor) or isinstance(far, torch.Tensor) or ray_live is not None
    plain = per_ray and grid is None and eps == 0.0 and ray_live is None
    pc = _PathCall(rays_o, rays_d, viewdirs, near, far, white_bkgd, num_levels, t_rand, u, opts, noise if plain else None, per_ray=True,
                   ray_live=ray_live)
    n, dev = pc.n, pc.dev
    if grid is not None and grid.device != dev:
        raise ValueError(f"{name}: the grid is on {grid.device}, the rays on {dev}")
    if not plain and (pc.op.noise_std > 0 or t_rand is not None):
        raise ValueError(f"{name}: inference only, density noise (noise_std > 0) and t_rand are refused")
    occ = grid.c_struct() if grid is not None else None
    occupied = torch.zeros(2, dtype=torch.int64, device=dev) if want_stats else None
    extra = (C.byref(occ) if occ is not None else None, _ptr(occupied))
    if occ_form and pc.bounds is None:
        stop, ws = None, _occ_workspace(dev, n, pc.st, workspace_bytes)
    else:
        stop = torch.zeros((n, 2), dtype=torch.int32, device=dev) if want_stats else None
        extra += (C.c_float(eps), R, _ptr(stop))
        if pc.bounds is not None:
            name, extra = name.rsplit("_", 1)[0] + "_bounds", extra + (C.byref(pc.bounds),)
        if plain:
            ws = torch.empty(int(workspace_bytes), dtype=torch.uint8, device=dev) if workspace_bytes is not None else _workspace(dev, n, pc.st)
        else:
            ws = _occ_workspace(dev, n, pc.st, workspace_bytes, "aon_render_stop_workspace_bytes")
    with torch.cuda.device(dev):
        check(getattr(lib, name)(*packs, *pc.args(ws), *extra), name)
    return (pc.outs, occupied) if occ_form else (pc.outs, occupied, stop)


def render_fwd_stop(packed_coarse, packed_fine, rays_o, rays_d, viewdirs, near, far, white_bkgd, grid, eps, round_samples=None, num_levels=2,
                    u=None, opts=None, workspace_bytes=None, ray_live=None):
    return _stop_call("aon_render_fwd_stop", (_pk(packed_coarse), _pk(packed_fine)), rays_o, rays_d, viewdirs, near, far, white_bkgd, grid, eps,
                      round_samples, num_levels, u, opts, workspace_bytes, ray_live=ray_live)


def art_render_fwd_stop(packed_c, small_c, packed_f, small_f, rays_o, rays_d, viewdirs, near, far, white_bkgd, grid, eps, round_samples=None,
                        num_levels=2, u=None, opts=None, workspace_bytes=None, ray_live=None):
    return _stop_call("aon_art_render_fwd_stop", (_pk(packed_c), _pk(small_c), _pk(packed_f), _pk(small_f)), rays_o, rays_d, viewdirs, near, far,
                      white_bkgd, grid, eps, round_samples, num_levels, u, opts, workspace_bytes, ray_live=ray_live)


SCENE_MAX_OBJECTS, SCENE_MAX_MERGED = 16, 4096
_SCENE_WS = StreamCache()


def check_pose(pose, what: str = "pose") -> torch.Tensor:
    m = torch.as_tensor(pose).detach().to(device="cpu", dtype=torch.float32)
    if tuple(m.shape) != (3, 4):
        raise ValueError(f"{what}: expected a (3, 4) object-to-world matrix, got shape {tuple(m.shape)}")
    R = m[:, :3].double()
    err = float((R.T @ R - torch.eye(3, dtype=torch.float64)).abs().max())
    if not err <= 1e-5:
        raise ValueError(f"{what}: the rotation is not orthonormal (max |R^T R - I| = {err:.3g} > 1e-5; scaled or sheared placements are not supported)")
    if not float(torch.linalg.det(R)) > 0:
        raise ValueError(f"{what}: the rotation has a negative determinant (a reflection)")
    return m.contiguous()


def _scene_objects(objects):
    objects = list(objects)
    if not 1 <= len(objects) <= SCENE_MAX_OBJECTS:
        raise ValueError(f"a scene holds 1 to {SCENE_MAX_OBJECTS} objects, got {len(objects)}")
    arr = (_lib.SceneObjectC * len(objects))()
    for k, ob in enumerate(objects):
        pose, box = (ob.pose, ob.box) if hasattr(ob, "pose") else ob
        m = check_pose(pose, f"object {k}: pose")
        lo, hi = _box3(box)
        arr[k].rot[:] = m[:, :3].reshape(-1).tolist()
        arr[k].centre[:] = m[:, 3].tolist()
        arr[k].lo[:] = list(lo)
        arr[k].hi[:] = list(hi)
    return arr, len(objects)


class ScenePairs:

    def __init__(self, n, K, offsets, counts, slot, ray, rays_o, rays_d, viewdirs, near, far):
        self.n, self.K, self.offsets, self.counts, self.slot = n, K, offsets, counts, slot
        self.starts = [sum(counts[:k]) for k in range(K + 1)]
        self.P = P = self.starts[K]
        self.capacity = {"ray": ray, "rays_o": rays_o, "rays_d": rays_d, "viewdirs": viewdirs, "near": near, "far": far}
        self.ray, self.rays_o, self.rays_d, self.viewdirs, self.near, self.far = ray[:P], rays_o[:P], rays_d[:P], viewdirs[:P], near[:P], far[:P]

    def segment(self, k: int) -> slice:
        return slice(self.starts[k], self.starts[k + 1])


def scene_pairs(rays_o, rays_d, viewdirs, objects) -> ScenePairs:
    o, d, v = (_f32(x.detach(), nm).reshape(-1, 3) for x, nm in ((rays_o, "rays_o"), (rays_d, "rays_d"), (viewdirs, "viewdirs")))
    n, dev = o.shape[0], o.device
    if d.shape[0] != n or v.shape[0] != n:
        raise ValueError("rays_o, rays_d and viewdirs must hold the same number of rays")
    arr, K = _scene_objects(objects)
    cap = n * K
    if n == 0:
        e = lambda *shape, dtype=torch.float32: torch.empty(shape, dtype=dtype, device=dev)
        return ScenePairs(0, K, torch.zeros((K + 1,), dtype=torch.int64, device=dev), [0] * K, e(0, K, dtype=torch.int32), e(0, dtype=torch.int32),
                          e(0, 3), e(0, 3), e(0, 3), e(0), e(0))
    offsets = torch.empty((K + 1,), dtype=torch.int64, device=dev)
    slot = torch.empty((n, K), dtype=torch.int32, device=dev)
    ray = torch.empty((cap,), dtype=torch.int32, device=dev)
    po, pd, pv = (torch.empty((cap, 3), dtype=torch.float32, device=dev) for _ in range(3))
    near, far = (torch.empty((cap,), dtype=torch.float32, device=dev) for _ in range(2))
    ws = _scratch(_SCENE_WS, dev, int(lib.aon_scene_pairs_workspace_bytes(n, K)))
    with torch.cuda.device(dev):
# ... 98 lines not shown
```

include/aon_hip.h:

```cpp
#ifndef AON_HIP_H
#define AON_HIP_H

#include <stdint.h>

#ifdef __cplusplus
extern "C" {
#endif

#define AON_ABI_VERSION 5

#define AON_OK 0
#define AON_E_INVALID (-1)
#define AON_E_WORKSPACE (-2)
#define AON_E_HIP_BASE (-1000)

#define AON_ACT_NONE 0
#define AON_ACT_VANILLA 1
#define AON_ACT_ARTICULATED 2

int aon_abi_version(void);
const char* aon_last_error(void);

int aon_raygen(const float* c2w_host, int H, int W, float focal, int64_t pix_begin, int64_t pix_end,
               float* rays_o, float* viewdirs, float* rays_d, void* stream);
// ... 116 lines not shown
                      float* dplanes, int64_t Np, void* stream);
int aon_vanilla_wgrad(const float* planes, const float* dplanes, const float* d_raw, int64_t Np,
                      float* const* grads_host, void* workspace, int64_t workspace_bytes, void* stream, const void* packed_bwd);
int aon_wgrad_plan(int articulated, int64_t Np, int cus, int32_t* jobs6, int max_jobs, int64_t* ws_bytes);
int aon_wgrad_plan_segment(int articulated, int64_t Np, int cus, int job, int workgroup, int32_t* begin_end);
int aon_set_wgrad_probe(void* device_buffer);
int aon_wgrad_kind_bench(int kind, int nlayers, const float* planes, const float* dplanes, int rows, int64_t Np, void* workspace,
                         int64_t workspace_bytes, void* stream);

int64_t aon_art_train_plane_rows(void);
int64_t aon_art_train_mask_bytes(int64_t Np);
int64_t aon_art_bwd_packed_bytes(void);
int aon_pack_art_mlp_bwd(const float* const* params_host, void* packed_bwd, void* stream);
int aon_pack_art_mlp_bwd_deg(const float* const* params_host, int min_deg_point, int max_deg_point, int deg_view, void* packed_bwd, void* stream);
int aon_art_mlp_fwd_train(const void* packed, const void* small, const float* rays_o, const float* rays_d,
                          const float* viewdirs, const float* t_vals, int64_t n_rays, int S, float* raw, float* planes,
                          void* masks, void* stream);
int aon_art_bwd_chain(const void* packed_bwd, const void* small, const float* d_raw, const void* masks,
                      const float* planes, float* dplanes, float* dxp, int64_t Np, void* stream);
int aon_art_wgrad(const float* planes, const float* dplanes, const float* d_raw, const float* dxp, int64_t Np,
                  const float* const* params_host, const float* shape, const float* appearance,
                  const float* articulation, float* const* grads_host, float* g_shape, float* g_appearance,
                  float* g_articulation, void* workspace, int64_t workspace_bytes, void* stream, const void* packed_bwd);
int aon_art_wgrad_deg(const float* planes, const float* dplanes, const float* d_raw, const float* dxp, int64_t Np,
                      const float* const* params_host, const float* shape, const float* appearance,
                      const float* articulation, float* const* grads_host, float* g_shape, float* g_appearance,
                      float* g_articulation, void* workspace, int64_t workspace_bytes, void* stream, int min_deg_point,
                      int max_deg_point, int deg_view, const void* packed_bwd);

int aon_set_bwd_overlap(int on);
int aon_set_fwd_overlap(int on);
int aon_set_fwd_merge(int on);
int aon_set_bwd_merge(int on);
int aon_set_bwd_early_heads(int on);
int aon_set_view_bias(int on);
int aon_get_view_bias(void);
int aon_view_bias(const void* packed, const float* viewdirs, int64_t n_rays, float* view_bias, void* stream);
int64_t aon_train_workspace_bytes(int64_t n_rays, int articulated, int num_levels);
int64_t aon_train_scratch_bytes(int64_t n_rays, int articulated, int num_levels);
int aon_render_fwd_train(const void* packed_coarse, const void* packed_fine, const float* rays_o, const float* rays_d,
                         const float* viewdirs, int64_t n_rays, float near_, float far_, int white_bkgd, int num_levels,
                         const float* t_rand, const float* u, int64_t u_stride, float* rgb_c, float* acc_c, float* depth_c,
                         float* rgb_f, float* acc_f, float* depth_f, void* workspace, int64_t workspace_bytes, void* stream);
int aon_render_bwd(const void* packed_bwd_coarse, const void* packed_fwd_coarse, const void* packed_bwd_fine,
                   const void* packed_fwd_fine, const float* rays_d, int64_t n_rays, int white_bkgd, int num_levels,
                   const float* const* g_rgb_host, const float* const* g_acc_host, const float* const* g_depth_host,
                   float* const* grads_coarse_host, float* const* grads_fine_host, void* workspace,
                   int64_t workspace_bytes, void* scratch, int64_t scratch_bytes, void* stream);
int aon_art_render_fwd_train(const void* packed_coarse, const void* small_coarse, const void* packed_fine,
                             const void* small_fine, const float* rays_o, const float* rays_d, const float* viewdirs,
                             int64_t n_rays, float near_, float far_, int white_bkgd, int num_levels, const float* t_rand,
                             const float* u, int64_t u_stride, float* rgb_c, float* acc_c, float* depth_c, float* rgb_f,
                             float* acc_f, float* depth_f, void* workspace, int64_t workspace_bytes, void* stream);
int aon_art_render_bwd(const void* packed_bwd_coarse, const void* small_coarse, const void* packed_bwd_fine,
                       const void* small_fine, const float* rays_d, int64_t n_rays, int white_bkgd, int num_levels,
                       const float* const* g_rgb_host, const float* const* g_acc_host, const float* const* g_depth_host,
                       const float* const* params_coarse_host, const float* const* params_fine_host, const float* shape,
                       const float* appearance, const float* articulation, float* const* grads_coarse_host,
                       float* const* grads_fine_host, float* g_shape, float* g_appearance, float* g_articulation,
                       void* workspace, int64_t workspace_bytes, void* scratch, int64_t scratch_bytes, void* stream);

typedef struct aon_render_opts {
  int32_t num_coarse_samples;
  int32_t num_fine_samples;
  int32_t lindisp;
  float inv_near, inv_far;
  float noise_std;
  const float* noise_c;
  const float* noise_f;
  float rgb_scale, rgb_shift, sigma_bias;
  int32_t min_deg_point, max_deg_point, deg_view;
} aon_render_opts;
void aon_render_opts_init(aon_render_opts* opts);

int aon_sample_along_rays_ex(const float* rays_o, const float* rays_d, int64_t n_rays, int S, float near_, float far_, int lindisp,
                             float inv_near, float inv_far, const float* t_rand, float* t_vals, float* coords, void* stream);
int aon_composite_ex(const float* rgb, int rgb_stride, const float* sigma, int sigma_stride, const float* t_vals, const float* dirs,
                     int64_t n_rays, int S, int white_bkgd, int act, const aon_render_opts* opts, float* comp_rgb, float* acc,
                     float* depth, float* weights, void* stream);
int aon_sample_pdf_n(const float* bins, const float* weights, int64_t w_stride, const float* t_coarse, const float* u,
                     int64_t u_stride, int64_t n_rays, int num_bins, int num_samples, int num_t, float* samples, float* t_fine,
                     void* stream);
int64_t aon_render_workspace_bytes_ex(int64_t n_rays, const aon_render_opts* opts);
int aon_render_fwd_ex(const void* packed_coarse, const void* packed_fine, const float* rays_o, const float* rays_d,
                      const float* viewdirs, int64_t n_rays, float near_, float far_, int white_bkgd, int num_levels,
                      const float* t_rand, const float* u, int64_t u_stride, float* rgb_c, float* acc_c, float* depth_c,
                      float* rgb_f, float* acc_f, float* depth_f, void* workspace, int64_t workspace_bytes, void* stream,
                      const aon_render_opts* opts);
int aon_art_render_fwd_ex(const void* packed_coarse, const void* small_coarse, const void* packed_fine, const void* small_fine,
                          const float* rays_o, const float* rays_d, const float* viewdirs, int64_t n_rays, float near_, float far_,
                          int white_bkgd, int num_levels, const float* t_rand, const float* u, int64_t u_stride, float* rgb_c,
                          float* acc_c, float* depth_c, float* rgb_f, float* acc_f, float* depth_f, void* workspace,
                          int64_t workspace_bytes, void* stream, const aon_render_opts* opts);
typedef struct aon_occupancy {
  const uint32_t* bits;
  int64_t cells[3];
  float lo[3];
  float step[3];
} aon_occupancy;
int64_t aon_occupancy_bytes(const int64_t* cells3_host);
int aon_occupancy_build(const float* density, const int64_t* dims3_host, float threshold, int dilate, uint32_t* bits, void* stream);
int64_t aon_render_occ_workspace_bytes(int64_t n_rays, const aon_render_opts* opts);
int aon_render_fwd_occ(const void* packed_coarse, const void* packed_fine, const float* rays_o, const float* rays_d,
                       const float* viewdirs, int64_t n_rays, float near_, float far_, int white_bkgd, int num_levels,
                       const float* t_rand, const float* u, int64_t u_stride, float* rgb_c, float* acc_c, float* depth_c,
                       float* rgb_f, float* acc_f, float* depth_f, void* workspace, int64_t workspace_bytes, void* stream,
                       const aon_render_opts* opts, const aon_occupancy* occ, int64_t* occupied_dev);
int aon_art_render_fwd_occ(const void* packed_coarse, const void* small_coarse, const void* packed_fine, const void* small_fine,
                           const float* rays_o, const float* rays_d, const float* viewdirs, int64_t n_rays, float near_, float far_,
                           int white_bkgd, int num_levels, const float* t_rand, const float* u, int64_t u_stride, float* rgb_c,
                           float* acc_c, float* depth_c, float* rgb_f, float* acc_f, float* depth_f, void* workspace,
                           int64_t workspace_bytes, void* stream, const aon_render_opts* opts, const aon_occupancy* occ,
                           int64_t* occupied_dev);
int64_t aon_render_stop_workspace_bytes(int64_t n_rays, const aon_render_opts* opts);
int aon_render_fwd_stop(const void* packed_coarse, const void* packed_fine, const float* rays_o, const float* rays_d,
                        const float* viewdirs, int64_t n_rays, float near_, float far_, int white_bkgd, int num_levels,
                        const float* t_rand, const float* u, int64_t u_stride, float* rgb_c, float* acc_c, float* depth_c,
                        float* rgb_f, float* acc_f, float* depth_f, void* workspace, int64_t workspace_bytes, void* stream,
                        const aon_render_opts* opts, const aon_occupancy* occ, int64_t* occupied_dev, float eps, int round_samples,
                        int32_t* stop_dev);
int aon_art_render_fwd_stop(const void* packed_coarse, const void* small_coarse, const void* packed_fine, const void* small_fine,
                            const float* rays_o, const float* rays_d, const float* viewdirs, int64_t n_rays, float near_, float far_,
                            int white_bkgd, int num_levels, const float* t_rand, const float* u, int64_t u_stride, float* rgb_c,
                            float* acc_c, float* depth_c, float* rgb_f, float* acc_f, float* depth_f, void* workspace,
                            int64_t workspace_bytes, void* stream, const aon_render_opts* opts, const aon_occupancy* occ,
                            int64_t* occupied_dev, float eps, int round_samples, int32_t* stop_dev);
int64_t aon_train_workspace_bytes_ex(int64_t n_rays, int articulated, int num_levels, const aon_render_opts* opts);
int64_t aon_train_scratch_bytes_ex(int64_t n_rays, int articulated, int num_levels, const aon_render_opts* opts);
int aon_render_fwd_train_ex(const void* packed_coarse, const void* packed_fine, const float* rays_o, const float* rays_d,
                            const float* viewdirs, int64_t n_rays, float near_, float far_, int white_bkgd, int num_levels,
                            const float* t_rand, const float* u, int64_t u_stride, float* rgb_c, float* acc_c, float* depth_c,
                            float* rgb_f, float* acc_f, float* depth_f, void* workspace, int64_t workspace_bytes, void* stream,
                            const aon_render_opts* opts);
int aon_render_bwd_ex(const void* packed_bwd_coarse, const void* packed_fwd_coarse, const void* packed_bwd_fine,
                      const void* packed_fwd_fine, const float* rays_d, int64_t n_rays, int white_bkgd, int num_levels,
                      const float* const* g_rgb_host, const float* const* g_acc_host, const float* const* g_depth_host,
                      float* const* grads_coarse_host, float* const* grads_fine_host, void* workspace,
                      int64_t workspace_bytes, void* scratch, int64_t scratch_bytes, void* stream, const aon_render_opts* opts);
int aon_art_render_fwd_train_ex(const void* packed_coarse, const void* small_coarse, const void* packed_fine,
                                const void* small_fine, const float* rays_o, const float* rays_d, const float* viewdirs,
                                int64_t n_rays, float near_, float far_, int white_bkgd, int num_levels, const float* t_rand,
                                const float* u, int64_t u_stride, float* rgb_c, float* acc_c, float* depth_c, float* rgb_f,
                                float* acc_f, float* depth_f, void* workspace, int64_t workspace_bytes, void* stream,
                                const aon_render_opts* opts);
int aon_art_render_bwd_ex(const void* packed_bwd_coarse, const void* small_coarse, const void* packed_bwd_fine,
                          const void* small_fine, const float* rays_d, int64_t n_rays, int white_bkgd, int num_levels,
                          const float* const* g_rgb_host, const float* const* g_acc_host, const float* const* g_depth_host,
                          const float* const* params_coarse_host, const float* const* params_fine_host, const float* shape,
                          const float* appearance, const float* articulation, float* const* grads_coarse_host,
                          float* const* grads_fine_host, float* g_shape, float* g_appearance, float* g_articulation,
                          void* workspace, int64_t workspace_bytes, void* scratch, int64_t scratch_bytes, void* stream,
                          const aon_render_opts* opts);
int64_t aon_train_scratch_bytes_latents(int64_t n_rays, int num_levels, const aon_render_opts* opts);
int aon_art_render_bwd_latents(const void* packed_bwd_coarse, const void* small_coarse, const void* packed_bwd_fine,
                               const void* small_fine, const float* rays_d, int64_t n_rays, int white_bkgd, int num_levels,
                               const float* const* g_rgb_host, const float* const* g_acc_host, const float* const* g_depth_host,
                               const float* const* params_coarse_host, const float* const* params_fine_host, float* g_shape,
                               float* g_appearance, float* g_articulation, void* workspace, int64_t workspace_bytes,
                               void* scratch, int64_t scratch_bytes, void* stream, const aon_render_opts* opts);
typedef struct aon_ray_grads {
  const float* rays_o; const float* viewdirs;
  float* g_rays_o; float* g_rays_d; float* g_viewdirs;
} aon_ray_grads;
int64_t aon_train_scratch_bytes_inputs(int64_t n_rays, int num_levels, const aon_render_opts* opts);
int aon_art_render_bwd_inputs(const void* packed_bwd_coarse, const void* small_coarse, const void* packed_bwd_fine,
                              const void* small_fine, const float* rays_d, int64_t n_rays, int white_bkgd, int num_levels,
// ... 89 lines not shown
```

Baseline: 540,800 rays/s.

## Defer view-branch MLP to compacted list of samples with positive density

Splits the vanilla inference MLP into a trunk kernel that writes sigma and stores the 256-wide trunk features only for samples with sigma>0, then compacts those samples and runs the view/RGB branch only on them. Samples with zero density contribute nothing to compositing, so their RGB head is skipped. It processes rays in slabs of up to 32768 to bound the extra feature buffer (1 KB per live sample). In exchange it adds a global round trip of trunk activations, a compaction pass and extra launches per slab.

```diff
diff --git a/articulated-object-nerf_amd/_lib.py b/articulated-object-nerf_amd/_lib.py
--- a/articulated-object-nerf_amd/_lib.py
+++ b/articulated-object-nerf_amd/_lib.py
@@ -124,6 +124,10 @@
     "aon_set_bwd_early_heads": (_i, [_i]),
     "aon_set_view_bias": (_i, [_i]),
     "aon_get_view_bias": (_i, []),
+    "aon_set_deferred_view": (_i, [_i]),
+    "aon_get_deferred_view": (_i, []),
+    "aon_render_deferred_workspace_bytes": (_l, [_l, _p]),
+    "aon_test_set_deferred_slab": (_i, [_i]),
     "aon_view_bias": (_i, [_p, _p, _l, _p, _p]),
     "aon_set_bwd_overlap": (_i, [_i]),
     "aon_set_fwd_overlap": (_i, [_i]),
diff --git a/articulated-object-nerf_amd/csrc/aon_capi.hip b/articulated-object-nerf_amd/csrc/aon_capi.hip
--- a/articulated-object-nerf_amd/csrc/aon_capi.hip
+++ b/articulated-object-nerf_amd/csrc/aon_capi.hip
@@ -24,6 +24,7 @@
 
 std::atomic<int> g_fuse_coarse{1};
 std::atomic<int> g_view_bias{1};
+std::atomic<int> g_deferred_view{1};
 
 const char* make_geo(const aon_render_opts* o, Geo& g, bool general_engine) {
   aon_render_opts d;
@@ -679,6 +680,13 @@
 }
 
 int aon_get_view_bias(void) { return g_view_bias.load(std::memory_order_relaxed); }
+
+int aon_set_deferred_view(int on) {
+  g_deferred_view.store(on ? 1 : 0, std::memory_order_relaxed);
+  return AON_OK;
+}
+
+int aon_get_deferred_view(void) { return g_deferred_view.load(std::memory_order_relaxed); }
 
 int64_t aon_art_packed_bytes(void) { return aon::art_stream_bytes(); }
 int64_t aon_art_small_bytes(void) { return aon::art_small_bytes(); }
diff --git a/articulated-object-nerf_amd/csrc/aon_capi_render.hip b/articulated-object-nerf_amd/csrc/aon_capi_render.hip
--- a/articulated-object-nerf_amd/csrc/aon_capi_render.hip
+++ b/articulated-object-nerf_amd/csrc/aon_capi_render.hip
@@ -13,10 +13,22 @@
   float* vbias;
   char* occ;
   char* stop;
+  int64_t slab; uint8_t* live_mark; char* live_list; float* live_rows;
   int64_t bytes;
 };
 
-Ws carve(char* base, int64_t n, const Geo& g, bool occ = false, bool stop = false) {
+int64_t defer_bytes(int64_t s, const Geo& g) {
+  return s <= 0 ? 0 : align_up(s * g.Sf, 256) + aon::occ_list_bytes(s * g.Sf) + align_up(s * g.Sf * 1024, 256);
+}
+std::atomic<int> g_defer_slab_test{0};
+constexpr int64_t kDeferSlabRays = 32768, kDeferMinSlabRays = 4096;
+int64_t defer_slab_cap(const Geo& g) {
+  if (const int t = g_defer_slab_test.load(std::memory_order_relaxed); t > 0) return t;
+  const int64_t by_rows = ((int64_t)8 << 30) / ((int64_t)g.Sf * 1024);
+  return by_rows < kDeferSlabRays ? (by_rows < 1 ? 1 : by_rows) : kDeferSlabRays;
+}
+
+Ws carve(char* base, int64_t n, const Geo& g, bool occ = false, bool stop = false, int64_t slab = 0) {
   Ws w{};
   int64_t off = 0;
   w.t_c = reinterpret_cast<float*>(base + off); off += align_up(n * g.Sc * 4, 256);
@@ -32,6 +44,12 @@
   }
   if (occ) { w.occ = base + off; off += aon::occ_list_bytes(n * g.Sf); }
   if (stop) { w.stop = base + off; off += aon::occ_stop_state_bytes(n); }
+  if (slab > 0) {
+    w.slab = slab;
+    w.live_mark = reinterpret_cast<uint8_t*>(base + off); off += align_up(slab * g.Sf, 256);
+    w.live_list = base + off; off += aon::occ_list_bytes(slab * g.Sf);
+    w.live_rows = reinterpret_cast<float*>(base + off); off += align_up(slab * g.Sf * 1024, 256);
+  }
   w.bytes = off;
   return w;
 }
@@ -49,6 +67,20 @@
 }
 int64_t aon_render_workspace_bytes_ex(int64_t n_rays, const aon_render_opts* opts) { return workspace_query(n_rays, opts, false, false); }
 int64_t aon_render_workspace_bytes(int64_t n_rays) { return aon_render_workspace_bytes_ex(n_rays, nullptr); }
+int64_t aon_render_deferred_workspace_bytes(int64_t n_rays, const aon_render_opts* opts) {
+  const int64_t plain = workspace_query(n_rays, opts, false, false);
+  if (plain < 0) return plain;
+  Geo g;
+  (void)make_geo(opts, g);
+  if (g.other_degrees) return plain;
+  if (n_rays < 1) n_rays = 1;
+  const int64_t cap = defer_slab_cap(g);
+  return plain + defer_bytes(n_rays < cap ? n_rays : cap, g);
+}
+int aon_test_set_deferred_slab(int rays) {
+  g_defer_slab_test.store(rays > 0 ? rays : 0, std::memory_order_relaxed);
+  return AON_OK;
+}
 
 
 struct NetRef {
@@ -127,6 +159,24 @@
   MlpTimer timer(stream, n * S);
   if (net.articulated)
     return aon::launch_art_mlp_fwd(static_cast<const char*>(net.packed), net.small, o, d, v, t, n, S, raw, stream, vbias);
+  if (w && w->slab > 0 && vbias && !(g->noise[level] && g->noise_std > 0.f)) {
+    const char* packed = static_cast<const char*>(net.packed);
+    for (int64_t r = 0; r < n; r += w->slab) {
+      const int64_t ns = n - r < w->slab ? n - r : w->slab;
+      float* raw_s = raw + r * S * 4;
+      if (hipError_t e = aon::launch_mlp_trunk_defer(packed, o + r * 3, d + r * 3, v + r * 3, t + r * S, ns, S, raw_s, w->live_mark, w->live_rows, stream);
+          e != hipSuccess) return e;
+      const int64_t starts[2] = {0, ns * S};
+      const aon::OccGrid no_grid{};
+      const aon::OccCompact c{&no_grid, starts, 1, 1, 0, 1, nullptr, nullptr, nullptr, w->live_mark, nullptr};
+      const int* live_idx = nullptr;
+      const int64_t* live_count = nullptr;
+      if (hipError_t e = aon::launch_occ_compact(c, nullptr, w->live_list, (ns * S + 1023) / 1024, nullptr, &live_idx, &live_count, stream); e != hipSuccess) return e;
+      if (hipError_t e = aon::launch_view_deferred(packed, w->live_rows, live_idx, live_count, ns * S, vbias + r * aon::kCondWidth, S, raw_s, stream);
+          e != hipSuccess) return e;
+    }
+    return hipSuccess;
+  }
   return aon::launch_mlp_fwd(static_cast<const char*>(net.packed), o, d, v, t, n, S, raw, stream, vbias);
 }
 
@@ -159,7 +209,18 @@
                                                 : with_occ ? "render: workspace smaller than aon_render_occ_workspace_bytes(1)"
                                                          : "render: workspace smaller than aon_render_workspace_bytes(1)");
   }
-  const Ws w = carve(static_cast<char*>(c.workspace), chunk, g, with_occ, with_stop);
+  int64_t slab = 0;
+  if (!art && !with_occ && !g.other_degrees && g_deferred_view.load(std::memory_order_relaxed) != 0) {
+    const int64_t left = c.workspace_bytes - carve(nullptr, chunk, g).bytes;
+    int64_t s = defer_slab_cap(g) < chunk ? defer_slab_cap(g) : chunk;
+    if (defer_bytes(s, g) > left) {
+      s = left / ((int64_t)g.Sf * 1030);
+      while (s > 0 && defer_bytes(s, g) > left) --s;
+    }
+    const bool hook = g_defer_slab_test.load(std::memory_order_relaxed) > 0;
+    if (s > 0 && (hook || s >= kDeferMinSlabRays || s >= chunk)) slab = s;
+  }
+  const Ws w = carve(static_cast<char*>(c.workspace), chunk, g, with_occ, with_stop, slab);
   if (with_occ && occ->tally) {
     if (int rc = check(hipMemsetAsync(occ->tally, 0, 2 * sizeof(int64_t), stream), who); rc != AON_OK) return rc;
   }
diff --git a/articulated-object-nerf_amd/csrc/aon_capi_util.h b/articulated-object-nerf_amd/csrc/aon_capi_util.h
--- a/articulated-object-nerf_amd/csrc/aon_capi_util.h
+++ b/articulated-object-nerf_amd/csrc/aon_capi_util.h
@@ -29,6 +29,7 @@
 
 extern std::atomic<int> g_fuse_coarse;
 extern std::atomic<int> g_view_bias;
+extern std::atomic<int> g_deferred_view;
 
 enum KClass { kMlpFwd = AON_PROF_MLP_FWD, kBwdChain = AON_PROF_BWD_CHAIN, kWgrad = AON_PROF_WGRAD, kComposite = AON_PROF_COMPOSITE,
               kSamplePdf = AON_PROF_SAMPLE_PDF, kCompositeBwd = AON_PROF_COMPOSITE_BWD, kCompositePdf = AON_PROF_COMPOSITE_PDF, kSampleT = AON_PROF_SAMPLE_T,
diff --git a/articulated-object-nerf_amd/csrc/aon_launch.h b/articulated-object-nerf_amd/csrc/aon_launch.h
--- a/articulated-object-nerf_amd/csrc/aon_launch.h
+++ b/articulated-object-nerf_amd/csrc/aon_launch.h
@@ -9,6 +9,10 @@
 void vanilla_fold_jobs_fwd(const float* const* params, float* packed, int view_levels, FoldGemm jobs[2]);
 hipError_t launch_mlp_fwd(const char* packed, const float* rays_o, const float* rays_d, const float* viewdirs,
                           const float* t_vals, int64_t n_rays, int S, float* raw, hipStream_t stream, const float* view_bias = nullptr);
+hipError_t launch_mlp_trunk_defer(const char* packed, const float* rays_o, const float* rays_d, const float* viewdirs, const float* t_vals,
+                                  int64_t n_rays, int S, float* raw, uint8_t* live_mark, float* live_rows, hipStream_t stream);
+hipError_t launch_view_deferred(const char* packed, const float* live_rows, const int* idx, const int64_t* count, int64_t max_listed,
+                                const float* view_bias, int S, float* raw, hipStream_t stream);
 hipError_t launch_view_bias(const char* packed, const float* viewdirs, int64_t n_rays, float* out, hipStream_t stream);
 hipError_t launch_view_bias_raw(const float* chunk, const float* bias_vec, const float* viewdirs, int64_t n_rays, float* out, hipStream_t stream);
 hipError_t launch_mlp_fwd_enc(const char* packed, const float* samples_enc, const float* viewdirs_enc, int64_t n_rays,
diff --git a/articulated-object-nerf_amd/csrc/aon_mlp.hip b/articulated-object-nerf_amd/csrc/aon_mlp.hip
--- a/articulated-object-nerf_amd/csrc/aon_mlp.hip
+++ b/articulated-object-nerf_amd/csrc/aon_mlp.hip
@@ -20,6 +20,13 @@
   static constexpr int kNumChunks = aon::kNumChunksF - 1;
   static constexpr int chunk_bytes(int c) { return aon::chunk_bytes_f(c < kChFView ? c : c + 1); }
   static constexpr int skip_before(int c) { return c == kChFView ? kSmallChunkBytes : 0; }
+};
+
+struct VanillaTrunkNet {
+  static constexpr int kSlotBytes = kPairSlotBytes;
+  static constexpr bool kPair = true;
+  static constexpr int kNumChunks = kChBott;
+  static constexpr int chunk_bytes(int) { return kBigChunkBytes; }
 };
 
 struct PackArgs {
@@ -97,10 +104,12 @@
   union {
     float* planes;
     const int* gather_idx;
+    float* live_rows;
   };
   union {
     u32x4* masks;
     const int64_t* gather_count;
+    uint8_t* live_mark;
   };
   int64_t Np;
   const float* view_bias;
@@ -121,11 +130,12 @@
   static constexpr int plane(int l) { return plane_h(l); }
 };
 
-template <bool ENC_IN_KERNEL, bool TRAIN, bool FOLD, bool VB = false, bool GATHER = false>
+template <bool ENC_IN_KERNEL, bool TRAIN, bool FOLD, bool VB = false, bool GATHER = false, bool DEFER = false>
 __global__ void __launch_bounds__(256) mlp_fwd_kernel(MlpArgs args) {
   static_assert(FOLD || !VB, "the per-ray view bias belongs to the folded form");
   static_assert(!GATHER || (ENC_IN_KERNEL && !TRAIN), "the occupancy list serves the inference kernel on in-kernel encodings");
-  using Net = std::conditional_t<VB, VanillaFoldVbNet, std::conditional_t<FOLD, VanillaFoldNet, VanillaNet>>;
+  static_assert(!DEFER || (ENC_IN_KERNEL && !TRAIN && VB && !GATHER), "the deferred view branch serves the dense per-ray-bias inference form");
+  using Net = std::conditional_t<DEFER, VanillaTrunkNet, std::conditional_t<VB, VanillaFoldVbNet, std::conditional_t<FOLD, VanillaFoldNet, VanillaNet>>>;
   const int tid = threadIdx.x;
   const int lane = tid & 63, wave = tid >> 6;
   const int m = lane & 31, h = lane >> 5;
@@ -179,7 +189,7 @@
       }
     };
     auto l7_side = [&](auto plain) {
-      if constexpr (VB) {
+      if constexpr (VB && !DEFER) {
         asm volatile("" : "+v"(ray32));
         return view_bias_side(plain, sg.view_bias + (int64_t)ray32 * kCondWidth + 4 * h, Z);
       } else {
@@ -187,43 +197,65 @@
       }
     };
     const float sigma = trunk_fwd<Net, VanillaTrunk>(p, E, X, Y, sm, h, taps, reread_enc, l7_side);
-    constexpr int kChV = FOLD ? kChFView : kChView;
-    auto reencode_view = [&]() {
-      if constexpr (TRAIN && ENC_IN_KERNEL) {
-        asm volatile("" : "+v"(vd[0]), "+v"(vd[1]), "+v"(vd[2]));
-        encode_view(vd, h, V);
-      }
-      if constexpr (TRAIN && !ENC_IN_KERNEL) {
-        int64_t rq = ray;
-        asm volatile("" : "+v"(rq));
-        load_view_enc(sg.viewdirs_enc + rq * kViewEnc, h, V);
-      }
-    };
-    if constexpr (FOLD) {
-      if constexpr (!VB) {
+    if constexpr (DEFER) {
+      const bool live = sigma > 0.f;
+      if (valid) {
+        if (h == 0) {
+          f32x4 o; o[0] = 0.f; o[1] = 0.f; o[2] = 0.f; o[3] = sigma;
+          reinterpret_cast<f32x4*>(sg.raw)[g] = o;
+          sg.live_mark[g] = live ? 1 : 0;
+        }
+        if (live) {
+          char* row = reinterpret_cast<char*>(sg.live_rows) + g * 1024 + h * 16;
+#pragma unroll
+          for (int t = 0; t < 8; ++t) {
+#pragma unroll
+            for (int q = 0; q < 4; ++q) {
+              f32x4 v; v[0] = Y[t][4 * q]; v[1] = Y[t][4 * q + 1]; v[2] = Y[t][4 * q + 2]; v[3] = Y[t][4 * q + 3];
+              __builtin_nontemporal_store(v, reinterpret_cast<f32x4*>(row + (32 * t + 8 * q) * 4));
+            }
+          }
+        }
+      }
+    } else {
+      constexpr int kChV = FOLD ? kChFView : kChView;
+      auto reencode_view = [&]() {
+        if constexpr (TRAIN && ENC_IN_KERNEL) {
+          asm volatile("" : "+v"(vd[0]), "+v"(vd[1]), "+v"(vd[2]));
+          encode_view(vd, h, V);
+        }
+        if constexpr (TRAIN && !ENC_IN_KERNEL) {
+          int64_t rq = ray;
+          asm volatile("" : "+v"(rq));
+          load_view_enc(sg.viewdirs_enc + rq * kViewEnc, h, V);
+        }
+      };
+      if constexpr (FOLD) {
+        if constexpr (!VB) {
+          init_bias(Z, sm + kSmBiasView, h);
+          reencode_view();
+          chunk_mma<Net, kChV, 4, 14>(p, V, Z);
+        }
+        dense_layer<Net, kChV + (VB ? 0 : 1), 8, 4>(p, Y, Z, taps.consume(Y, plane_h(7), true)); taps.put_mask(7);
+      } else {
+        init_bias(X, sm + kSmBiasBott, h); dense_layer<Net, kChBott, 8, 8>(p, Y, X, taps.consume(Y, plane_h(7), true)); taps.put_mask(7);
         init_bias(Z, sm + kSmBiasView, h);
+        dense_layer<Net, kChV, 8, 4>(p, X, Z, taps.consume(X, kPlBot, false));
         reencode_view();
-        chunk_mma<Net, kChV, 4, 14>(p, V, Z);
-      }
-      dense_layer<Net, kChV + (VB ? 0 : 1), 8, 4>(p, Y, Z, taps.consume(Y, plane_h(7), true)); taps.put_mask(7);
-    } else {
-      init_bias(X, sm + kSmBiasBott, h); dense_layer<Net, kChBott, 8, 8>(p, Y, X, taps.consume(Y, plane_h(7), true)); taps.put_mask(7);
-      init_bias(Z, sm + kSmBiasView, h);
-      dense_layer<Net, kChV, 8, 4>(p, X, Z, taps.consume(X, kPlBot, false));
-      reencode_view();
-      chunk_mma<Net, kChV + 8, 4, 14>(p, V, Z);
-    }
-    relu_tiles(Z);
-    taps.burst(Z, kPlHV, 8);
-    float rgb[3];
-#pragma unroll
-    for (int ch = 0; ch < 3; ++ch) {
-      float v = head_partial<4>(Z, sm + kSmWRgb + ch * kCondWidth, h);
-      rgb[ch] = v + __shfl_xor(v, 32) + sm[kSmBRgb + ch];
-    }
-    if (valid && h == 0) {
-      f32x4 o; o[0] = rgb[0]; o[1] = rgb[1]; o[2] = rgb[2]; o[3] = sigma;
-      reinterpret_cast<f32x4*>(sg.raw)[g] = o;
+        chunk_mma<Net, kChV + 8, 4, 14>(p, V, Z);
+      }
+      relu_tiles(Z);
+      taps.burst(Z, kPlHV, 8);
+      float rgb[3];
+#pragma unroll
+      for (int ch = 0; ch < 3; ++ch) {
+        float v = head_partial<4>(Z, sm + kSmWRgb + ch * kCondWidth, h);
+        rgb[ch] = v + __shfl_xor(v, 32) + sm[kSmBRgb + ch];
+      }
+      if (valid && h == 0) {
+        f32x4 o; o[0] = rgb[0]; o[1] = rgb[1]; o[2] = rgb[2]; o[3] = sigma;
+        reinterpret_cast<f32x4*>(sg.raw)[g] = o;
+      }
     }
   });
 }
@@ -267,10 +299,10 @@
   return cus;
 }
 
-template <bool ENC, bool TRAIN, bool FOLD, bool VB = false, bool GATHER = false>
+template <bool ENC, bool TRAIN, bool FOLD, bool VB = false, bool GATHER = false, bool DEFER = false>
 static hipError_t launch_mlp_tf(const MlpArgs& args, hipStream_t stream) {
   static DeviceOnce lds_once;
-  return launch_persistent(&mlp_fwd_kernel<ENC, TRAIN, FOLD, VB, GATHER>, kLdsBytes, args.npass_total, lds_once, stream, args);
+  return launch_persistent(&mlp_fwd_kernel<ENC, TRAIN, FOLD, VB, GATHER, DEFER>, kLdsBytes, args.npass_total, lds_once, stream, args);
 }
 
 template <bool ENC, bool TRAIN, bool GATHER = false>
@@ -332,6 +364,128 @@
                               viewdirs, n_rays, out, stream);
 }
 
+struct ViewArgs {
+  const char* packed;
+  const float* rows;
+  const int* idx;
+  const int64_t* count;
+  const float* view_bias;
+  float* raw;
+  int S;
+};
+constexpr int kViewWBytes = 8 * kSmallChunkBytes;
+constexpr int kViewLdsBytes = kViewWBytes + (int)kSmallBytes;
+
+__device__ __forceinline__ int view_listed(const ViewArgs& a, int64_t listed, int64_t tile, int m) {
+  const int64_t e = tile * 32 + m;
+  return a.idx[e < listed ? e : listed - 1];
+}
+__device__ __forceinline__ void view_gather_tile(const ViewArgs& a, int g, int h, int t, f32x16& Y) {
+  const char* row = reinterpret_cast<const char*>(a.rows) + (int64_t)g * 1024 + h * 16;
+#pragma unroll
+  for (int q = 0; q < 4; ++q) {
+    const f32x4 v = *reinterpret_cast<const f32x4*>(row + (32 * t + 8 * q) * 4);
+    Y[4 * q] = v[0]; Y[4 * q + 1] = v[1]; Y[4 * q + 2] = v[2]; Y[4 * q + 3] = v[3];
+  }
+}
+__device__ __forceinline__ void view_bias_init(const ViewArgs& a, int g, int h, f32x16 (&Z)[4]) {
+  const float* vb = a.view_bias + (int64_t)(g / a.S) * kCondWidth + 4 * h;
+#pragma unroll
+  for (int i = 0; i < 16; ++i) {
+    const f32x4 v = *reinterpret_cast<const f32x4*>(vb + 32 * (i >> 2) + 8 * (i & 3));
+    Z[i >> 2][4 * (i & 3)] = v[0]; Z[i >> 2][4 * (i & 3) + 1] = v[1]; Z[i >> 2][4 * (i & 3) + 2] = v[2]; Z[i >> 2][4 * (i & 3) + 3] = v[3];
+  }
+}
+__device__ __forceinline__ void view_chunk(const char* w, int j, int lane, const f32x16& Y, f32x16 (&Z)[4], const f32x16 (&Z0)[4]) {
+  const char* buf = w + j * kSmallChunkBytes + lane * 16;
+#pragma unroll
+  for (int i = 0; i < 16; ++i) {
+    const int q = i / 4, tp = i % 4;
+    const f32x4 av = *reinterpret_cast<const f32x4*>(buf + i * 1024);
+#pragma unroll
+    for (int cc = 0; cc < 4; ++cc)
+      Z[tp] = __builtin_amdgcn_mfma_f32_32x32x2f32(av[cc], Y[4 * q + cc], (j == 0 && q == 0 && cc == 0) ? Z0[tp] : Z[tp], 0, 0, 0);
+  }
+}
+
+__global__ void __launch_bounds__(256) view_kernel(ViewArgs a) {
+  extern __shared__ __attribute__((aligned(16))) char smem[];
+  const int64_t listed = *a.count;
+  const int64_t ntiles = (listed + 31) / 32;
+  if ((int64_t)blockIdx.x * 4 >= ntiles) return;
+  float* sm = reinterpret_cast<float*>(smem + kViewWBytes);
+  {
+    const f32x4* src = reinterpret_cast<const f32x4*>(a.packed + chunk_offset_f(kChFView + 1));
+    f32x4* dst = reinterpret_cast<f32x4*>(smem);
+    for (int i = threadIdx.x; i < kViewWBytes / 16; i += 256) dst[i] = src[i];
+  }
+  load_small_block<kSmallFloats>(sm, reinterpret_cast<const float*>(a.packed + kStreamBytes));
+  __syncthreads();
+  const int lane = threadIdx.x & 63, m = lane & 31, h = lane >> 5;
+  const int wave = __builtin_amdgcn_readfirstlane(threadIdx.x >> 6);
+  const int64_t stride = (int64_t)gridDim.x * 4;
+  int64_t tile = (int64_t)blockIdx.x * 4 + wave;
+  if (tile >= ntiles) return;
+  f32x16 Y[8], Z[4], Zb[4];
+  int g = view_listed(a, listed, tile, m);
+  int gn = view_listed(a, listed, tile + stride, m);
+  __builtin_amdgcn_sched_barrier(0);
+  view_bias_init(a, g, h, Zb);
+  __builtin_amdgcn_sched_barrier(0);
+#pragma unroll
+  for (int t = 0; t < 8; ++t) view_gather_tile(a, g, h, t, Y[t]);
+  __builtin_amdgcn_sched_barrier(0);
+  while (true) {
+    const int64_t nxt = tile + stride;
+    const int gnn = view_listed(a, listed, nxt + stride, m);
+#pragma unroll
+    for (int j = 0; j < 8; ++j) {
+      view_chunk(smem, j, lane, Y[j], Z, Zb);
+      __builtin_amdgcn_sched_barrier(0);
+      view_gather_tile(a, gn, h, j, Y[j]);
+      if (j == 3) view_bias_init(a, gn, h, Zb);
+      __builtin_amdgcn_sched_barrier(0);
+    }
+    relu_tiles(Z);
+    float rgb[3];
+#pragma unroll
+    for (int ch = 0; ch < 3; ++ch) {
+      const float v = head_partial<4>(Z, sm + kSmWRgb + ch * kCondWidth, h);
+      rgb[ch] = v + __shfl_xor(v, 32) + sm[kSmBRgb + ch];
+    }
+    if (tile * 32 + m < listed && h == 0) {
+      float* rec = a.raw + (int64_t)g * 4;
+      rec[0] = rgb[0]; rec[1] = rgb[1]; rec[2] = rgb[2];
+    }
+    if (nxt >= ntiles) break;
+    tile = nxt; g = gn; gn = gnn;
+  }
+}
+
+hipError_t launch_mlp_trunk_defer(const char* packed, const float* rays_o, const float* rays_d, const float* viewdirs, const float* t_vals,
+                                  int64_t n_rays, int S, float* raw, uint8_t* live_mark, float* live_rows, hipStream_t stream) {
+  if (stream_form(packed) != kFormFolded) return hipErrorInvalidValue;
+  MlpArgs args{};
+  fill_seg(args.seg[0], TrainSeg{packed, nullptr, rays_o, rays_d, viewdirs, t_vals, n_rays, S, raw, nullptr, nullptr, 0, nullptr});
+  args.seg[0].live_rows = live_rows; args.seg[0].live_mark = live_mark;
+  finish_segs(args, 1);
+  return launch_mlp_tf<true, false, true, true, false, true>(args, stream);
+}
+
+hipError_t launch_view_deferred(const char* packed, const float* live_rows, const int* idx, const int64_t* count, int64_t max_listed,
+                                const float* view_bias, int S, float* raw, hipStream_t stream) {
+  if (stream_form(packed) != kFormFolded) return hipErrorInvalidValue;
+  if (max_listed <= 0) return hipSuccess;
+  static DeviceOnce lds_once;
+  if (hipError_t e = set_max_lds(&view_kernel, kViewLdsBytes, lds_once); e != hipSuccess) return e;
+  const int cus = num_cus();
+  if (cus <= 0) return hipErrorInvalidDevice;
+  const int64_t groups = (max_listed + 127) / 128;
+  const ViewArgs a{packed, live_rows, idx, count, view_bias, raw, S};
+  view_kernel<<<dim3((unsigned)(groups < cus ? groups : cus)), dim3(256), kViewLdsBytes, stream>>>(a);
+  return hipGetLastError();
+}
+
 hipError_t launch_mlp_fwd(const char* packed, const float* rays_o, const float* rays_d, const float* viewdirs,
                           const float* t_vals, int64_t n_rays, int S, float* raw, hipStream_t stream, const float* view_bias) {
   MlpArgs args{};
@@ -384,13 +538,6 @@
   finish_segs(args, 1);
   return launch_mlp_t<false, false>(args, stream);
 }
-
-struct VanillaTrunkNet {
-  static constexpr int kSlotBytes = kPairSlotBytes;
-  static constexpr bool kPair = true;
-  static constexpr int kNumChunks = kChBott;
-  static constexpr int chunk_bytes(int) { return kBigChunkBytes; }
-};
 
 
 __global__ void __launch_bounds__(256) density_grid_kernel(GridArgs args) {
diff --git a/articulated-object-nerf_amd/csrc/aon_occ.hip b/articulated-object-nerf_amd/csrc/aon_occ.hip
--- a/articulated-object-nerf_amd/csrc/aon_occ.hip
+++ b/articulated-object-nerf_amd/csrc/aon_occ.hip
@@ -107,7 +107,7 @@
   sentinel[0] = 0.f; sentinel[1] = 0.f; sentinel[2] = 0.f; sentinel[3] = -__builtin_huge_valf();
 #pragma unroll
   for (int r = 0; r < kOccPer; ++r)
-    if (s.rec[r] >= 0 && !s.occ[r]) raw[s.rec[r]] = sentinel;
+    if (raw && s.rec[r] >= 0 && !s.occ[r]) raw[s.rec[r]] = sentinel;
   if (threadIdx.x == 0) {
     int tot = 0;
 #pragma unroll
diff --git a/articulated-object-nerf_amd/ops.py b/articulated-object-nerf_amd/ops.py
--- a/articulated-object-nerf_amd/ops.py
+++ b/articulated-object-nerf_amd/ops.py
@@ -532,13 +532,14 @@
 MAX_CHUNK_RAYS = 327680
 
 
-def _workspace(device, n_rays: int, st=None) -> torch.Tensor:
+def _workspace(device, n_rays: int, st=None, vanilla=False) -> torch.Tensor:
     chunk = MAX_CHUNK_RAYS
     if st is not None and (st.min_deg_point, st.max_deg_point, st.deg_view) != (0, 10, 4):
         chunk = 65536
-    need = int(lib.aon_render_workspace_bytes_ex(min(n_rays, chunk), None if st is None else C.byref(st)))
+    query = "aon_render_deferred_workspace_bytes" if vanilla and lib.aon_get_deferred_view() else "aon_render_workspace_bytes_ex"
+    need = int(getattr(lib, query)(min(n_rays, chunk), None if st is None else C.byref(st)))
     if need < 0:
-        check(need, "aon_render_workspace_bytes_ex")
+        check(need, query)
     return _scratch(_WS_CACHE, device, need)
 
 
@@ -586,7 +587,7 @@
         return _stop_call(name + "_stop", packs, rays_o, rays_d, viewdirs, near, far, white_bkgd, None, 0.0, None, num_levels, u, opts, workspace_bytes,
                           t_rand=t_rand, noise=noise, ray_live=ray_live, want_stats=False)[0]
     pc = _PathCall(rays_o, rays_d, viewdirs, near, far, white_bkgd, num_levels, t_rand, u, opts, noise)
-    ws = _workspace(pc.dev, pc.n, pc.st)
+    ws = _workspace(pc.dev, pc.n, pc.st, vanilla=name == "aon_render_fwd")
     with torch.cuda.device(pc.dev):
         check(getattr(lib, name + "_ex")(*packs, *pc.args(ws)), name)
     return pc.outs
@@ -932,6 +933,14 @@
 
 def set_view_bias(on: bool) -> None:
     check(lib.aon_set_view_bias(int(bool(on))), "aon_set_view_bias")
+
+
+def set_deferred_view(on: bool) -> None:
+    check(lib.aon_set_deferred_view(int(bool(on))), "aon_set_deferred_view")
+
+
+def deferred_view_enabled() -> bool:
+    return bool(lib.aon_get_deferred_view())
 
 
 def view_bias_enabled() -> bool:
@@ -1632,7 +1641,8 @@
         if pc.bounds is not None:
             name, extra = name.rsplit("_", 1)[0] + "_bounds", extra + (C.byref(pc.bounds),)
         if plain:
-            ws = torch.empty(int(workspace_bytes), dtype=torch.uint8, device=dev) if workspace_bytes is not None else _workspace(dev, n, pc.st)
+            ws = torch.empty(int(workspace_bytes), dtype=torch.uint8, device=dev) if workspace_bytes is not None else \
+                _workspace(dev, n, pc.st, vanilla=name.startswith("aon_render_fwd"))
         else:
             ws = _occ_workspace(dev, n, pc.st, workspace_bytes, "aon_render_stop_workspace_bytes")
     with torch.cuda.device(dev):
diff --git a/include/aon_hip.h b/include/aon_hip.h
--- a/include/aon_hip.h
+++ b/include/aon_hip.h
@@ -222,6 +222,10 @@
                      int64_t u_stride, int64_t n_rays, int num_bins, int num_samples, int num_t, float* samples, float* t_fine,
                      void* stream);
 int64_t aon_render_workspace_bytes_ex(int64_t n_rays, const aon_render_opts* opts);
+int aon_set_deferred_view(int on);
+int aon_get_deferred_view(void);
+int64_t aon_render_deferred_workspace_bytes(int64_t n_rays, const aon_render_opts* opts);
+int aon_test_set_deferred_slab(int rays);
 int aon_render_fwd_ex(const void* packed_coarse, const void* packed_fine, const float* rays_o, const float* rays_d,
                       const float* viewdirs, int64_t n_rays, float near_, float far_, int white_bkgd, int num_levels,
                       const float* t_rand, const float* u, int64_t u_stride, float* rgb_c, float* acc_c, float* depth_c,
```

New measurement: 548,000 rays/s, median of 6. 1.3% higher.
